# igashov/DiffLinker

Measured on NVIDIA H100. Metric: molecules/sec (T=500 denoising), higher is better.
Workload: dtype f32

## Files before the change

### difflinker_b200/csrc/common.cuh

```cuda
#pragma once
#include <cuda_runtime.h>
#include <stdint.h>

namespace dl {

constexpr int H = 128;
constexpr int MAX_DIN = 32;
constexpr int MAX_XHD = 16;

constexpr int OPT_TANH = 1;
constexpr int OPT_MEAN = 2;
constexpr int OPT_SIN = 4;
constexpr int N_SIN_FREQ = 6;
constexpr int N_SIN_FEAT = 4 * N_SIN_FREQ;
__device__ __forceinline__ float sin_freq(int k) { return __int_as_float(__float_as_int(0x1.aceeap-2f) + (k << 24)); }
__device__ __forceinline__ float sin_arg(float r, int k) { return __fmul_rn(__fsqrt_rn(__fadd_rn(r, 1e-8f)), sin_freq(k)); }
__device__ __forceinline__ float radial_rn(float dx, float dy, float dz) {
  return __fadd_rn(__fadd_rn(__fmul_rn(dx, dx), __fmul_rn(dy, dy)), __fmul_rn(dz, dz));
}

__device__ __forceinline__ void chain_wait() { asm volatile("griddepcontrol.wait;" ::: "memory"); }
__device__ __forceinline__ void chain_release() { asm volatile("griddepcontrol.launch_dependents;" ::: "memory"); }

inline bool& chain_overlap_enabled() { static bool on = true; return on; }

template <typename... KArgs, typename... Args>
inline cudaError_t launch_chain(void (*kernel)(KArgs...), dim3 grid, dim3 block, size_t smem, cudaStream_t st, Args&&... args) {
  cudaLaunchConfig_t cfg = {};
  cfg.gridDim = grid; cfg.blockDim = block; cfg.dynamicSmemBytes = smem; cfg.stream = st;
  cudaLaunchAttribute at[1];
  at[0].id = cudaLaunchAttributeProgrammaticStreamSerialization;
  at[0].val.programmaticStreamSerializationAllowed = chain_overlap_enabled() ? 1 : 0;
  cfg.attrs = at; cfg.numAttrs = 1;
  return cudaLaunchKernelEx(&cfg, kernel, KArgs(static_cast<Args&&>(args))...);
}

__device__ __forceinline__ float silu_f(float x) {
  float t, r;
  asm("ex2.approx.ftz.f32 %0, %1;" : "=f"(t) : "f"(x * -1.4426950408889634f));
  asm("rcp.approx.ftz.f32 %0, %1;" : "=f"(r) : "f"(1.0f + t));
  return x * r;
}

__device__ __forceinline__ float usig_f(float u) {
  float t, r;
  asm("ex2.approx.ftz.f32 %0, %1;" : "=f"(t) : "f"(u));
  asm("rcp.approx.ftz.f32 %0, %1;" : "=f"(r) : "f"(1.0f + t));
  return u * r;
}

__device__ __forceinline__ float2 fadd2(float2 a, float2 b) { return make_float2(__fadd_rn(a.x, b.x), __fadd_rn(a.y, b.y)); }
__device__ __forceinline__ float2 fmul2(float2 a, float2 b) { return make_float2(__fmul_rn(a.x, b.x), __fmul_rn(a.y, b.y)); }
__device__ __forceinline__ float2 ffma2(float2 a, float2 b, float2 c) { return make_float2(__fmaf_rn(a.x, b.x, c.x), __fmaf_rn(a.y, b.y, c.y)); }
__device__ __forceinline__ float ex2_approx(float x) { float y; asm("ex2.approx.ftz.f32 %0, %1;" : "=f"(y) : "f"(x)); return y; }
__device__ __forceinline__ float rcp_approx(float x) { float y; asm("rcp.approx.ftz.f32 %0, %1;" : "=f"(y) : "f"(x)); return y; }
__device__ __forceinline__ float2 sigmoid_pair_log2(float2 u) {
  const float2 den = fadd2(make_float2(ex2_approx(fminf(u.x, 63.0f)), ex2_approx(fminf(u.y, 63.0f))), make_float2(1.0f, 1.0f));
  const float r = rcp_approx(den.x * den.y);
  return fmul2(make_float2(r, r), make_float2(den.y, den.x));
}
__device__ __forceinline__ void usig4(float2 u01, float2 u23, float2& s01, float2& s23) {
  const float2 one = make_float2(1.0f, 1.0f);
  const float2 ab = fadd2(make_float2(ex2_approx(fminf(u01.x, 31.0f)), ex2_approx(fminf(u01.y, 31.0f))), one);
  const float2 cd = fadd2(make_float2(ex2_approx(fminf(u23.x, 31.0f)), ex2_approx(fminf(u23.y, 31.0f))), one);
  const float2 m = fmul2(ab, cd);
  const float r = rcp_approx(m.x * m.y);
  const float2 rm = fmul2(make_float2(r, r), make_float2(m.y, m.x));
  s01 = fmul2(u01, fmul2(rm, cd));
  s23 = fmul2(u23, fmul2(rm, ab));
}
__device__ __forceinline__ float2 usig2(float2 u) { return fmul2(u, sigmoid_pair_log2(u)); }
__device__ __forceinline__ float2 silu2(float2 x) {
  return fmul2(x, sigmoid_pair_log2(fmul2(x, make_float2(-1.4426950408889634f, -1.4426950408889634f))));
}

struct EdgeMlpW {
  const float* W1a_t;
  const float* W1b_t;
  const float* b1;
  const float* wd;
  const float* w0;
  const float* W2_t;
  const float* b2;
  const void* W2_tc;
  float w2_descale;
  float wdmax, w0max;
  const void* W1_tc;
  float w1_descale;
  const float* b1_u;
  const float* wd_u;
  const float* w0_u;
  const float* we;
  const float* we_u;
};

struct GclW : EdgeMlpW {
  const float* W3_t;
  const float* b3;
  const float* W4_t;
  const float* b4;
  const void* W3_tc;
  const void* W4_tc;
  float w3_descale, w4_descale;
};

struct EqW : EdgeMlpW {
  const float* w5;
};

struct ProjW {
  const float* W1a_t;
  const float* W1b_t;
  const float* b1;
};

struct Plan {
  const int* rowidx;
  const int* colidx;
  const int* xrowidx;
  const int* nr;
  const int* nc;
  const int* nxr;
  const int4* items;
  const int* n_items;
  const int* xmols;
  const int* n_xmols;
  const int4* xitems;
  const int* n_xitems;
};

struct Geom {
  int B, N;
  int F;
  int C;
  int D;
  int graph_type;
  float norm_constant;
  float normalization_factor;
};

}
```

### difflinker_b200/csrc/dl_engine.cu

```cuda
#include <cuda_fp16.h>
#include <cuda_runtime.h>

#include <algorithm>
#include <cmath>
#include <cstdarg>
#include <cstdio>
#include <cstdlib>
#include <cstring>
#include <ctime>
#include <map>
#include <string>
#include <vector>

#include "../../include/difflinker_b200.h"
#include "kernels_simt.cuh"
#include "kernels_tc.cuh"
#include "kernels_node_tc.cuh"
#include "kernels_retry.cuh"

using namespace dl;

static thread_local char g_err[1024] = "";
static void set_err(const char* fmt, ...) {
  va_list ap;
  va_start(ap, fmt);
  vsnprintf(g_err, sizeof(g_err), fmt, ap);
  va_end(ap);
}

#define CK(call)                                                                          \
  do {                                                                                    \
    cudaError_t _e = (call);                                                              \
    if (_e != cudaSuccess) {                                                              \
      set_err("%s:%d %s -> %s", __FILE__, __LINE__, #call, cudaGetErrorString(_e));       \
      return DL_ERR_CUDA;                                                                 \
    }                                                                                     \
  } while (0)

namespace {

struct Workspace {
  int B = 0, N = 0;
  float *nm = nullptr, *x0 = nullptr, *xa = nullptr, *xb = nullptr, *h = nullptr, *ABg = nullptr, *ABc = nullptr,
        *agg = nullptr, *z = nullptr, *ABgmax = nullptr, *ABcmax = nullptr, *eps = nullptr;
  int* cls = nullptr;
  int *nbr = nullptr, *recs = nullptr, *xrecs = nullptr, *n_recs = nullptr;
  float4 *x04 = nullptr, *xa4 = nullptr, *xb4 = nullptr;
  int *rowidx = nullptr, *colidx = nullptr, *xrowidx = nullptr, *nr = nullptr, *nc = nullptr, *nxr = nullptr,
      *n_items = nullptr, *xmols = nullptr, *n_xmols = nullptr, *n_xitems = nullptr;
  int4* items = nullptr;
  int4* xitems = nullptr;
  int* tile_ctr = nullptr;
  unsigned long long* seeds = nullptr;
  std::vector<void*> allocs;
};

struct HostStage {
  size_t cap = 0;
  char* buf = nullptr;
};

struct KernelTimes {
  bool on = false;
  struct Rec { const char* label; cudaEvent_t a, b; };
  std::vector<Rec> pending;
  std::map<std::string, std::pair<double, long>> acc;
  void begin(cudaStream_t st, const char* label) {
    if (!on) return;
    cudaStreamCaptureStatus cap = cudaStreamCaptureStatusNone;
    cudaStreamIsCapturing(st, &cap);
    if (cap != cudaStreamCaptureStatusNone) return;
    Rec r{label, nullptr, nullptr};
    cudaEventCreate(&r.a); cudaEventCreate(&r.b);
    cudaEventRecord(r.a, st);
    pending.push_back(r);
  }
  void end(cudaStream_t st) {
    if (!on || pending.empty() || pending.back().b == nullptr) return;
    cudaStreamCaptureStatus cap = cudaStreamCaptureStatusNone;
    cudaStreamIsCapturing(st, &cap);
    if (cap != cudaStreamCaptureStatusNone) return;
    cudaEventRecord(pending.back().b, st);
  }
  void collect(cudaStream_t st) {
    if (!on || pending.empty()) return;
    cudaStreamSynchronize(st);
    for (auto& r : pending) {
      float ms = 0.f;
      if (cudaEventElapsedTime(&ms, r.a, r.b) == cudaSuccess) { auto& a = acc[r.label]; a.first += ms; a.second += 1; }
      cudaEventDestroy(r.a); cudaEventDestroy(r.b);
    }
    pending.clear();
  }
  void report() {
    if (!on || acc.empty()) return;
    double tot = 0;
    for (auto& kv : acc) tot += kv.second.first;
    for (auto& kv : acc)
      fprintf(stderr, "[dl times] %-22s %6ld launches  avg %8.2f us  share %5.1f%%\n", kv.first.c_str(), kv.second.second,
              1e3 * kv.second.first / kv.second.second, 100.0 * kv.second.first / tot);
  }
};

}

struct dl_engine {
  dl_config cfg{};
  dl_egnn_options opts{};
  int D = 0;
  int num_sms = 0;
  int max_threads_per_sm = 2048;
  int slice_B_full = 0, slice_b0 = 0;
  int start_step = -1;
  float start_alpha = 0.f, start_sigma = 0.f;
  std::vector<int32_t> starts_t0;
  std::vector<float> starts_alpha, starts_sigma;
  HostStage start_rows;
  int resamplings = 1, resample_T = 0;
  std::vector<float> jump;
  std::vector<dl_step_coef> coef_passes;
  int64_t mol_steps = 0;
  bool finalized = false;
  std::map<std::string, std::vector<float>> raw;
  float* wblob = nullptr;
  __half* wblob_tc = nullptr;
  std::vector<GclW> gcl;
  std::vector<EqW> eq;
  const float *We_t = nullptr, *be = nullptr, *Wo = nullptr, *bo = nullptr;
  Workspace ws;
  Workspace ws_sub;
  HostStage sub_rows;
  HostStage hashes;
  bool ring_set = false;
  unsigned long long ring_allowed = 0;
  HostStage ring_masks;
  int ring_B = 0;
  HostStage anchors;
  bool anchors_set = false;
  int anchors_B = 0, anchors_N = 0;
  cudaEvent_t ev_r0 = nullptr, ev_r1 = nullptr, ev_g0 = nullptr, ev_g1 = nullptr;
  float retry_ms = 0.f;
  cudaStream_t loop_stream = nullptr;
  cudaEvent_t ev_in = nullptr, ev_out = nullptr, ev_t0 = nullptr, ev_t1 = nullptr;
  float* coef_dev = nullptr;
  int coef_cap = 0;
  int* step_ctr = nullptr;
  int64_t launches = 0;
  HostStage stage;
  KernelTimes times;
  bool use_tc = false;
  const int8_t* last_edge_mask = nullptr;
  const float* last_linker_mask = nullptr;
  int last_B = 0, last_N = 0;
};

namespace {

int edges_in(const dl_engine* e) { return e->opts.sin_embedding ? N_SIN_FEAT : 2; }

#define TIMED(label, stream, stmt) do { e->times.begin(stream, label); stmt; e->times.end(stream); } while (0)

struct ExpectedParam {
  std::string name;
  int64_t numel;
};

std::vector<ExpectedParam> expected_params(const dl_config& c, int edges_in) {
  const int D = c.in_node_nf + c.context_node_nf + (c.condition_time ? 1 : 0);
  const int Hh = c.hidden_nf;
  std::vector<ExpectedParam> v;
  v.push_back({"dynamics.embedding.weight", (int64_t)Hh * D});
  v.push_back({"dynamics.embedding.bias", Hh});
  v.push_back({"dynamics.embedding_out.weight", (int64_t)D * Hh});
  v.push_back({"dynamics.embedding_out.bias", D});
  char buf[160];
  for (int l = 0; l < c.n_layers; ++l) {
    for (int s = 0; s < c.inv_sublayers; ++s) {
      snprintf(buf, sizeof(buf), "dynamics.e_block_%d.gcl_%d.", l, s);
      std::string p(buf);
      v.push_back({p + "edge_mlp.0.weight", (int64_t)Hh * (2 * Hh + edges_in)});
      v.push_back({p + "edge_mlp.0.bias", Hh});
      v.push_back({p + "edge_mlp.2.weight", (int64_t)Hh * Hh});
      v.push_back({p + "edge_mlp.2.bias", Hh});
      v.push_back({p + "node_mlp.0.weight", (int64_t)Hh * 2 * Hh});
      v.push_back({p + "node_mlp.0.bias", Hh});
      v.push_back({p + "node_mlp.2.weight", (int64_t)Hh * Hh});
      v.push_back({p + "node_mlp.2.bias", Hh});
    }
    snprintf(buf, sizeof(buf), "dynamics.e_block_%d.gcl_equiv.", l);
    std::string p(buf);
    v.push_back({p + "coord_mlp.0.weight", (int64_t)Hh * (2 * Hh + edges_in)});
    v.push_back({p + "coord_mlp.0.bias", Hh});
    v.push_back({p + "coord_mlp.2.weight", (int64_t)Hh * Hh});
    v.push_back({p + "coord_mlp.2.bias", Hh});
    v.push_back({p + "coord_mlp.4.weight", Hh});
  }
  return v;
}

using RawWeights = std::map<std::string, std::vector<float>>;

struct Packer {
  std::vector<float> blob;
  std::vector<__half> tc;
  std::vector<std::pair<const float**, size_t>> fields;
  std::vector<std::pair<const void**, size_t>> tc_fields;
  void add(const float** field, const std::vector<float>& seg) {
    while (blob.size() % 4) blob.push_back(0.f);
    fields.push_back({field, blob.size()});
    blob.insert(blob.end(), seg.begin(), seg.end());
  }
  void add_tc(const void** field, size_t off) { tc_fields.push_back({field, off}); }
  void point(const float* base, const __half* tc_base) const {
    for (auto& f : fields) *f.first = base + f.second;
    for (auto& f : tc_fields) *f.first = tc_base + f.second;
  }
};

std::vector<float> transpose_block(const std::vector<float>& W, int out, int in_stride, int c0, int k) {
  std::vector<float> t((size_t)k * out);
  for (int o = 0; o < out; ++o)
    for (int i = 0; i < k; ++i) t[(size_t)i * out + o] = W[(size_t)o * in_stride + c0 + i];
  return t;
}
std::vector<float> column(const std::vector<float>& W, int out, int in_stride, int c) {
  std::vector<float> t(out);
  for (int o = 0; o < out; ++o) t[o] = W[(size_t)o * in_stride + c];
  return t;
}

void pack_edge_mlp(Packer& pk, EdgeMlpW& w, const RawWeights& raw, const std::string& p, int in1) {
  const auto& W1 = raw.at(p + "0.weight");
  pk.add(&w.W1a_t, transpose_block(W1, H, in1, 0, H));
  pk.add(&w.W1b_t, transpose_block(W1, H, in1, H, H));
  pk.add(&w.b1, raw.at(p + "0.bias"));
  pk.add(&w.wd, column(W1, H, in1, 2 * H));
  pk.add(&w.W2_t, transpose_block(raw.at(p + "2.weight"), H, H, 0, H));
  pk.add(&w.b2, raw.at(p + "2.bias"));
}

void pack_gcl(Packer& pk, GclW& w, const RawWeights& raw, const std::string& p, int in1) {
  pack_edge_mlp(pk, w, raw, p + "edge_mlp.", in1);
  pk.add(&w.W3_t, transpose_block(raw.at(p + "node_mlp.0.weight"), H, 2 * H, 0, 2 * H));
  pk.add(&w.b3, raw.at(p + "node_mlp.0.bias"));
  pk.add(&w.W4_t, transpose_block(raw.at(p + "node_mlp.2.weight"), H, H, 0, H));
  pk.add(&w.b4, raw.at(p + "node_mlp.2.bias"));
}

void pack_edge_mlp_denoiser(Packer& pk, EdgeMlpW& w, const RawWeights& raw, const std::string& p, bool sin_embedding) {
  const int IN1 = 2 * H + (sin_embedding ? N_SIN_FEAT : 2);
  auto scaled = [](const std::vector<float>& v) { std::vector<float> o(v.size()); for (size_t i = 0; i < v.size(); ++i) o[i] = (float)((double)v[i] * tc::NEG_LOG2E); return o; };
  auto absmax = [](const std::vector<float>& v) { float m = 0.f; for (float x : v) m = std::max(m, std::fabs(x)); return m; };
  const auto& W1 = raw.at(p + "0.weight");
  const std::vector<float> wd = column(W1, H, IN1, 2 * H), w0 = column(W1, H, IN1, 2 * H + 1);
  pk.add(&w.w0, w0);
  pk.add_tc(&w.W2_tc, tc::pack_w2(raw.at(p + "2.weight"), pk.tc, &w.w2_descale));
  pk.add_tc(&w.W1_tc, tcn::pack_blocks(scaled(W1), IN1, 2, pk.tc, &w.w1_descale));
  pk.add(&w.b1_u, scaled(raw.at(p + "0.bias")));
  pk.add(&w.wd_u, scaled(wd));
  pk.add(&w.w0_u, scaled(w0));
  w.wdmax = absmax(wd); w.w0max = absmax(w0);
  if (sin_embedding) {
    const std::vector<float> we = transpose_block(W1, H, IN1, 2 * H, N_SIN_FEAT);
    pk.add(&w.we, we);
    pk.add(&w.we_u, scaled(we));
    w.wdmax = 0.f; w.w0max = 0.f;
    for (int k = 0; k < N_SIN_FEAT; ++k) w.wdmax += absmax(std::vector<float>(we.begin() + k * H, we.begin() + (k + 1) * H));
  }
}

template <typename T>
dl_status upload_blob(const std::vector<T>& host, T** dev) {
  if (*dev) cudaFree(*dev);
  *dev = nullptr;
  CK(cudaMalloc((void**)dev, std::max<size_t>(host.size(), 1) * sizeof(T)));
  CK(cudaMemcpy(*dev, host.data(), host.size() * sizeof(T), cudaMemcpyHostToDevice));
  return DL_OK;
}

template <typename T>
dl_status dev_alloc(Workspace& ws, T** p, size_t count) {
  void* q = nullptr;
  CK(cudaMalloc(&q, std::max<size_t>(count, 1) * sizeof(T)));
  ws.allocs.push_back(q);
  *p = reinterpret_cast<T*>(q);
  return DL_OK;
}

void free_workspace(Workspace& ws) {
  for (void* p : ws.allocs) cudaFree(p);
  ws = Workspace();
}

dl_status ensure_workspace(dl_engine* e, int B, int N) {
  Workspace& ws = e->ws;
  if (ws.B == B && ws.N == N) return DL_OK;
  free_workspace(ws);
  const size_t n = (size_t)B * N;
  const int xd = 3 + e->cfg.in_node_nf;
  dl_status s;
#define WSA(field, cnt) if ((s = dev_alloc(ws, &ws.field, (cnt))) != DL_OK) return s
  WSA(nm, n); WSA(x0, n * 3); WSA(xa, n * 3); WSA(xb, n * 3); WSA(h, n * H); WSA(ABg, n * 2 * H); WSA(ABc, n * 2 * H);
  WSA(agg, n * H); WSA(z, n * xd); WSA(eps, n * xd); WSA(cls, n); WSA(x04, n); WSA(xa4, n); WSA(xb4, n); WSA(ABgmax, n * 2); WSA(ABcmax, n * 2);
  WSA(rowidx, n); WSA(colidx, n); WSA(xrowidx, n); WSA(nr, B); WSA(nc, B); WSA(nxr, B); WSA(n_items, 1);
  WSA(xmols, B); WSA(n_xmols, 1); WSA(items, n); WSA(xitems, n); WSA(n_xitems, 1); WSA(tile_ctr, 64); WSA(seeds, B);
  if (e->use_tc && e->cfg.graph_type != 0) { WSA(nbr, n * N); WSA(recs, n * CUT_REC); WSA(xrecs, n * CUT_REC); WSA(n_recs, 2); }
#undef WSA
  ws.B = B; ws.N = N;
  return DL_OK;
}

Plan make_plan(const Workspace& ws) {
  Plan p;
  p.rowidx = ws.rowidx; p.colidx = ws.colidx; p.xrowidx = ws.xrowidx; p.nr = ws.nr; p.nc = ws.nc; p.nxr = ws.nxr;
  p.items = ws.items; p.n_items = ws.n_items; p.xmols = ws.xmols; p.n_xmols = ws.n_xmols;
  p.xitems = ws.xitems; p.n_xitems = ws.n_xitems;
  return p;
}

Geom make_geom(const dl_engine* e, int B, int N) {
  Geom g;
  g.B = B; g.N = N; g.F = e->cfg.in_node_nf; g.C = e->cfg.context_node_nf; g.D = e->D;
  g.graph_type = e->cfg.graph_type; g.norm_constant = e->cfg.norm_constant;
  g.normalization_factor = e->cfg.normalization_factor;
  return g;
}

#define LAUNCH_CHECK()                                                                    \
  do {                                                                                    \
    cudaError_t _e = cudaGetLastError();                                                  \
    if (_e != cudaSuccess) {                                                              \
      set_err("%s:%d kernel launch -> %s", __FILE__, __LINE__, cudaGetErrorString(_e));   \
      return DL_ERR_CUDA;                                                                 \
    }                                                                                     \
  } while (0)

constexpr int PLAN_MAX_N = 48 * 1024 / (2 * (int)sizeof(int));

dl_status build_plan(Workspace& ws, int B, int N, int graph_type, const int8_t* node_mask, const float* linker_mask,
                     const int8_t* edge_mask, int tile_edges, int max_rows, cudaStream_t st) {
  if (N > PLAN_MAX_N) {
    set_err("N = %d exceeds the work plan's limit of %d rows per molecule", N, PLAN_MAX_N);
    return DL_ERR_UNSUPPORTED;
  }
  CK(cudaMemsetAsync(ws.agg, 0, (size_t)B * N * H * sizeof(float), st));
  k_plan_mol<<<B, 256, 2 * N * sizeof(int), st>>>(N, graph_type, edge_mask, node_mask, linker_mask, ws.rowidx,
                                                  ws.colidx, ws.xrowidx, ws.nr, ws.nc, ws.nxr);
  LAUNCH_CHECK();
  k_plan_items<<<1, 1, 0, st>>>(B, tile_edges, max_rows, 1, max_rows, ws.nr, ws.nc, ws.nxr, ws.items, ws.n_items, ws.xmols,
                                ws.n_xmols, ws.xitems, ws.n_xitems);
  LAUNCH_CHECK();
  return DL_OK;
}

dl_status build_forward_plan(dl_engine* e, int B, int N, const int8_t* node_mask, const float* linker_mask,
                             const int8_t* edge_mask, cudaStream_t st) {
  const dl_status s = build_plan(e->ws, B, N, e->cfg.graph_type, node_mask, linker_mask, edge_mask,
                                 e->use_tc ? tc::TN : ET, e->use_tc ? tc::MAXR : MAXR, st);
  if (s == DL_OK) e->launches += 2;
  return s;
}

struct FwdIO {
  const float* xh = nullptr; const float* t = nullptr; int t_numel = 0; float* out = nullptr;
  const int8_t* node_mask = nullptr; const float* linker_mask = nullptr; const int8_t* edge_mask = nullptr;
  const float* context = nullptr; int* nan_flags = nullptr;
  bool sampler = false; bool inpaint = false; const float* xh0 = nullptr; const float* upd_linker_mask = nullptr;
  const float* fragment_mask = nullptr; const float* noise = nullptr; float* chain = nullptr;
  NoiseRng rng{};
  int T = 0; float norm0 = 1.f, norm1 = 1.f, bias1 = 0.f;
  RowStarts rows{};
  int R = 1; const float* jump = nullptr;
};

ProjW proj_of(const EdgeMlpW& w) { return ProjW{w.W1a_t, w.W1b_t, w.b1}; }

EdgeArgs edge_args(const dl_engine* e, const EdgeMlpW& w, bool coord, const int8_t* edge_mask, const float* linker_mask,
                   const float* x, const float4* x4, float* x_out = nullptr, float4* x4_out = nullptr,
                   const float* w5 = nullptr) {
  const Workspace& ws = e->ws;
  const float ksc = e->use_tc ? 1.4426950408889634f : 1.0f;
  EdgeArgs ea{};
  ea.AB = coord ? ws.ABc : ws.ABg; ea.ABmax = coord ? ws.ABcmax : ws.ABgmax;
  ea.w2_descale = w.w2_descale; ea.wdmax = w.wdmax * ksc; ea.w0max = w.w0max * ksc;
  ea.x = x; ea.x0 = ws.x0; ea.x4 = x4; ea.x04 = ws.x04; ea.x4_out = x4_out;
  ea.edge_mask = edge_mask; ea.cls = ws.cls; ea.nm = ws.nm; ea.linker_mask = linker_mask;
  ea.W2_t = w.W2_t; ea.b2 = w.b2; ea.wd = e->use_tc ? w.wd_u : w.wd; ea.w0 = e->use_tc ? w.w0_u : w.w0; ea.w5 = w5;
  ea.plan = make_plan(ws); ea.agg = coord ? nullptr : ws.agg; ea.x_out = x_out; ea.nbr = ws.nbr;
  ea.recs = coord ? ws.xrecs : ws.recs;
  ea.n_recs = coord && ws.n_recs ? ws.n_recs + 1 : ws.n_recs;
  ea.coords_range = e->opts.coords_range;
  ea.we = e->use_tc ? w.we_u : w.we;
  return ea;
}

int edge_opt(const dl_engine* e, bool coord) {
  return (coord && e->opts.tanh ? OPT_TANH : 0) | (e->opts.aggregation == DL_AGGR_MEAN ? OPT_MEAN : 0) |
         (e->opts.sin_embedding ? OPT_SIN : 0);
}

struct NodeConsumer { const EdgeMlpW* w; float* AB; float* ABmax; };
int node_consumers(const dl_engine* e, int l, int s, NodeConsumer c[2]) {
  const int L = e->cfg.n_layers, S = e->cfg.inv_sublayers;
  const Workspace& ws = e->ws;
  if (s + 1 < S) { c[0] = {&e->gcl[l * S + s + 1], ws.ABg, ws.ABgmax}; return 1; }
  c[0] = {&e->eq[l], ws.ABc, ws.ABcmax};
  if (l + 1 == L) return 1;
  c[1] = {&e->gcl[(l + 1) * S], ws.ABg, ws.ABgmax};
  return 2;
}

tcn::NodeTcArgs node_tc_args(const dl_engine* e, const GclW& w, int l, int s) {
  const Workspace& ws = e->ws;
  tcn::NodeTcArgs ta{};
  ta.h = ws.h; ta.agg = ws.agg; ta.nm = ws.nm; ta.proj_only = s < 0;
  ta.w3 = reinterpret_cast<const __half*>(w.W3_tc); ta.w4 = reinterpret_cast<const __half*>(w.W4_tc);
  ta.b3 = w.b3; ta.b4 = w.b4; ta.w3_descale = w.w3_descale; ta.w4_descale = w.w4_descale;
  NodeConsumer c[2];
  ta.n_proj = node_consumers(e, l, s, c);
  for (int i = 0; i < ta.n_proj; ++i) {
    ta.pw[i] = reinterpret_cast<const __half*>(c[i].w->W1_tc); ta.pb1[i] = c[i].w->b1_u;
    ta.p_descale[i] = c[i].w->w1_descale; ta.AB[i] = c[i].AB; ta.ABmax[i] = c[i].ABmax;
  }
  ta.tile_nodes = tcn::pick_tile_nodes(ws.B * ws.N, e->num_sms);
  return ta;
}

template <bool COORD, int OPT = 0>
void launch_edge_simt(int opt, int num_sms, const Geom& gm, const EdgeArgs& ea, cudaStream_t st) {
  if constexpr (OPT <= (OPT_TANH | OPT_MEAN | OPT_SIN)) {
    if constexpr (COORD || !(OPT & OPT_TANH))
      if (opt == OPT) { k_edge_simt<COORD, ACT_SILU, OPT><<<num_sms, 256, EDGE_SIMT_SMEM, st>>>(gm, ea); return; }
    launch_edge_simt<COORD, OPT + 1>(opt, num_sms, gm, ea, st);
  }
}

template <bool COORD, int OPT = 0>
cudaError_t opt_in_edge_simt() {
  if constexpr (OPT > (OPT_TANH | OPT_MEAN | OPT_SIN)) {
    return cudaSuccess;
  } else {
    if constexpr (COORD || !(OPT & OPT_TANH)) {
      const cudaError_t err = cudaFuncSetAttribute(k_edge_simt<COORD, ACT_SILU, OPT>, cudaFuncAttributeMaxDynamicSharedMemorySize,
                                                   (int)EDGE_SIMT_SMEM);
      if (err != cudaSuccess) return err;
    }
    return opt_in_edge_simt<COORD, OPT + 1>();
  }
}

dl_status launch_edge(dl_engine* e, const Geom& gm, const EdgeArgs& ea, bool coord, const void* w2_tc, cudaStream_t st) {
  const int opt = edge_opt(e, coord);
  if (e->use_tc) {
    dl_status s = tc::launch_edge_tc(gm, ea, coord, opt, w2_tc, e->num_sms, st);
    if (s != DL_OK) { set_err("no tensor-core edge kernel for graph type %d with options %d", gm.graph_type, opt); return s; }
  } else if (coord) {
    launch_edge_simt<true>(opt, e->num_sms, gm, ea, st);
  } else {
    launch_edge_simt<false>(opt, e->num_sms, gm, ea, st);
  }
  LAUNCH_CHECK();
  e->launches += 1;
  return DL_OK;
}

dl_status enqueue_forward(dl_engine* e, int B, int N, const FwdIO& io, cudaStream_t st) {
  Workspace& ws = e->ws;
  const Geom gm = make_geom(e, B, N);
  const int n = B * N;
  const int L = e->cfg.n_layers, S = e->cfg.inv_sublayers;
  const int node_blocks = (n + NODE_TM - 1) / NODE_TM;
  const size_t node_smem = 3 * NODE_TM * LDX * sizeof(float);

  PrepArgs pa{};
  pa.xh = io.sampler ? ws.z : io.xh;
  pa.node_mask = io.node_mask; pa.linker_mask = io.linker_mask;
  pa.t = io.t; pa.t_numel = io.t_numel; pa.context = io.context;
  pa.We_t = e->We_t; pa.be = e->be; pa.proj = proj_of(e->gcl[0]);
  pa.nm = ws.nm; pa.x0 = ws.x0; pa.x = ws.xa; pa.x04 = e->use_tc ? ws.x04 : nullptr; pa.x4 = e->use_tc ? ws.xa4 : nullptr; pa.cls = ws.cls; pa.h = ws.h;
  pa.AB = e->use_tc ? nullptr : ws.ABg; pa.ABmax = ws.ABgmax;
  pa.coef = io.sampler ? e->coef_dev : nullptr;
  pa.step_prep = io.sampler ? e->step_ctr : nullptr;
  pa.step_fin = io.sampler ? e->step_ctr + 1 : nullptr;
  TIMED("k_prep", st, (launch_chain(k_prep, dim3(node_blocks), dim3(256), 0, st, gm, pa)));
  LAUNCH_CHECK();
  e->launches += 1;
  if (e->use_tc) {
    const tcn::NodeTcArgs ta = node_tc_args(e, e->gcl[0], 0, -1);
    TIMED("k_node_tc(proj only)", st, (tcn::launch_node(n, ta, st)));
    LAUNCH_CHECK();
    e->launches += 1;
  }

  if (ws.nbr != nullptr) {
    CK(cudaMemsetAsync(ws.n_recs, 0, 2 * sizeof(int), st));
    k_nbr<<<B, 512, (size_t)N * CUT_SMEM_PER_NODE, st>>>(N, e->cfg.graph_type, ws.x04, ws.cls, ws.rowidx, ws.colidx,
                                                        ws.xrowidx, ws.nr, ws.nc, ws.nxr, ws.nbr, ws.recs, ws.xrecs,
                                                        ws.n_recs);
    LAUNCH_CHECK();
    e->launches += 1;
  }

  float* xin = ws.xa;
  float* xout = ws.xb;
  float4* xin4 = ws.xa4;
  float4* xout4 = ws.xb4;
  e->last_edge_mask = io.edge_mask; e->last_linker_mask = io.linker_mask; e->last_B = B; e->last_N = N;
  for (int l = 0; l < L; ++l) {
    for (int s = 0; s < S; ++s) {
      const GclW& w = e->gcl[l * S + s];
      const EdgeArgs ea = edge_args(e, w, false, io.edge_mask, io.linker_mask, xin, xin4);
      e->times.begin(st, "edge GCL");
      dl_status st2 = launch_edge(e, gm, ea, false, w.W2_tc, st);
      e->times.end(st);
      if (st2 != DL_OK) return st2;

      if (e->use_tc) {
        const tcn::NodeTcArgs ta = node_tc_args(e, w, l, s);
        TIMED(ta.n_proj == 2 ? "k_node_tc(2 proj)" : "k_node_tc(1 proj)", st, (tcn::launch_node(n, ta, st)));
      } else {
        NodeArgs na{};
        na.h = ws.h; na.agg = ws.agg; na.nm = ws.nm; na.W3_t = w.W3_t; na.b3 = w.b3; na.W4_t = w.W4_t; na.b4 = w.b4;
        NodeConsumer c[2];
        const int n_proj = node_consumers(e, l, s, c);
        na.proj1 = proj_of(*c[0].w); na.AB1 = c[0].AB; na.ABmax1 = c[0].ABmax;
        if (n_proj == 2) { na.proj2 = proj_of(*c[1].w); na.AB2 = c[1].AB; na.ABmax2 = c[1].ABmax; }
        k_node<ACT_SILU><<<node_blocks, 256, node_smem, st>>>(n, na);
      }
      LAUNCH_CHECK();
      e->launches += 1;
    }
    k_copy_x<<<(n * 3 + 255) / 256, 256, 0, st>>>(n * 3, xin, xout, e->use_tc ? xin4 : nullptr, xout4);
    LAUNCH_CHECK();
    e->launches += 1;
    const EqW& w = e->eq[l];
    const EdgeArgs ea = edge_args(e, w, true, io.edge_mask, io.linker_mask, xin, xin4, xout, xout4, w.w5);
    e->times.begin(st, "edge COORD");
    dl_status st2 = launch_edge(e, gm, ea, true, w.W2_tc, st);
    e->times.end(st);
    if (st2 != DL_OK) return st2;
    std::swap(xin, xout);
    std::swap(xin4, xout4);
  }

  FinishArgs fa{};
  fa.h = ws.h; fa.x = xin; fa.x0 = ws.x0; fa.nm = ws.nm; fa.Wo = e->Wo; fa.bo = e->bo;
  fa.nan_flags = io.nan_flags;
  const bool fused_update = io.sampler && !io.inpaint;
  fa.out = fused_update ? nullptr : (io.sampler ? ws.eps : io.out);
  if (fused_update) {
    fa.z = ws.z; fa.fragment_mask = io.fragment_mask; fa.linker_mask = io.linker_mask; fa.noise = io.noise; fa.rng = io.rng;
    fa.coef = e->coef_dev; fa.step_fin = e->step_ctr + 1; fa.step_prep = e->step_ctr; fa.T = io.T;
    fa.norm0 = io.norm0; fa.norm1 = io.norm1; fa.bias1 = io.bias1; fa.chain = io.chain; fa.rows = io.rows;
  } else if (io.sampler) {
    fa.tag_step = e->step_ctr + (io.R > 1 ? 2 : 1);
  }
  const bool per_mol = io.rng.on == NOISE_PER_MOLECULE;
  TIMED("k_finish", st, (launch_chain(per_mol ? k_finish<true> : k_finish<false>, dim3((n + 15) / 16), dim3(256), 0, st, gm, fa)));
  LAUNCH_CHECK();
  e->launches += 1;
  if (e->cfg.centering || io.inpaint) {
    InpaintArgs ia{};
    ia.mode = io.inpaint ? 1 : 0;
    ia.eps = io.inpaint ? ws.eps : io.out; ia.nm = ws.nm; ia.z = ws.z; ia.xh0 = io.xh0;
    ia.fragment_mask = io.fragment_mask; ia.linker_mask = io.upd_linker_mask; ia.noise = io.noise; ia.rng = io.rng;
    ia.coef = e->coef_dev;
    ia.step_prep = e->step_ctr; ia.step_fin = e->step_ctr + 1; ia.T = io.T;
    ia.norm0 = io.norm0; ia.norm1 = io.norm1; ia.bias1 = io.bias1; ia.chain = io.chain;
    ia.R = io.R; ia.jump = io.jump; ia.step_tag = e->step_ctr + 2;
    if (io.R > 1) {
      if (per_mol) k_inpaint<true, true><<<B, 256, 0, st>>>(gm, ia);
      else k_inpaint<false, true><<<B, 256, 0, st>>>(gm, ia);
    } else if (per_mol) k_inpaint<true><<<B, 256, 0, st>>>(gm, ia);
    else k_inpaint<false><<<B, 256, 0, st>>>(gm, ia);
    LAUNCH_CHECK();
    e->launches += 1;
  }
  return DL_OK;
}

dl_status check_shapes(const dl_engine* e, int B, int N) {
  if (!e || !e->finalized) { set_err("engine not finalized (dl_finalize_weights)"); return DL_ERR_INVALID; }
  if (B <= 0 || N <= 0) { set_err("B and N must be positive (got %d, %d)", B, N); return DL_ERR_INVALID; }
  if ((int64_t)B * N * N > (int64_t)1 << 40) { set_err("B*N*N too large"); return DL_ERR_INVALID; }
  if (e->use_tc && e->cfg.graph_type != 0 && N > 4000) {
    set_err("cut-off graphs: N = %d exceeds the neighbour-list kernel's shared-memory staging (N <= 4000)", N);
    return DL_ERR_INVALID;
  }
  return DL_OK;
}

size_t align256(size_t v) { return (v + 255) & ~(size_t)255; }

struct StageLayout {
  struct Buf { const void* src; size_t bytes, off; bool used; };
  std::vector<Buf> bufs;
  size_t total = 0;
  char* base = nullptr;
  int add(const void* src, size_t bytes, bool used) {
    bufs.push_back({src, bytes, total, used});
    total += used ? align256(bytes) : 0;
    return (int)bufs.size() - 1;
  }
  int in(const void* src, size_t bytes) { return add(src, bytes, src != nullptr); }
  int out(size_t bytes) { return add(nullptr, bytes, true); }
  template <typename T> T* at(int i) const { return bufs[i].used ? reinterpret_cast<T*>(base + bufs[i].off) : nullptr; }
};

dl_status stage_inputs(HostStage& sg, StageLayout& sl, cudaStream_t st) {
  if (sg.cap < sl.total) {
    if (sg.buf) cudaFree(sg.buf);
    sg.buf = nullptr; sg.cap = 0;
    CK(cudaMalloc((void**)&sg.buf, sl.total));
    sg.cap = sl.total;
  }
  sl.base = sg.buf;
  for (const auto& b : sl.bufs)
    if (b.src) CK(cudaMemcpyAsync(sl.base + b.off, b.src, b.bytes, cudaMemcpyHostToDevice, st));
  return DL_OK;
}

dl_status stage_results(void* out, const void* d_out, size_t bytes, const int32_t* d_flags, int B, int32_t* nan_flags,
                        cudaStream_t st) {
  std::vector<int32_t> flags(B);
  CK(cudaMemcpyAsync(out, d_out, bytes, cudaMemcpyDeviceToHost, st));
  CK(cudaMemcpyAsync(flags.data(), d_flags, B * 4, cudaMemcpyDeviceToHost, st));
  CK(cudaStreamSynchronize(st));
  bool any = false;
  for (int i = 0; i < B; ++i) { any |= flags[i] != 0; if (nan_flags) nan_flags[i] = flags[i]; }
  return any ? DL_NAN_DETECTED : DL_OK;
}

dl_status check_slice(const dl_engine* e, int B) {
  if (e->slice_B_full > 0 && e->slice_b0 + B > e->slice_B_full) {
    set_err("batch slice [%d, %d) exceeds the full batch %d", e->slice_b0, e->slice_b0 + B, e->slice_B_full);
    return DL_ERR_INVALID;
  }
  return DL_OK;
}

dl_status check_sampler(const dl_engine* e, int sampler, int T, int keep_frames, bool has_draws, const float* xh,
                        const int8_t* node_mask, const float* fragment_mask, const float* linker_mask, const float* context,
                        const dl_step_coef* coef, const float* norm, const float* chain) {
  if (sampler != DL_SAMPLER_LINKER && sampler != DL_SAMPLER_INPAINT) { set_err("unknown sampler %d", sampler); return DL_ERR_INVALID; }
  if ((sampler == DL_SAMPLER_INPAINT) != (e->cfg.centering != 0)) { set_err("the inpainting sampler needs a model built with centering=1 (and vice versa)"); return DL_ERR_INVALID; }
  if (!xh || !node_mask || !fragment_mask || !linker_mask || !has_draws || !coef || !norm || !chain) {
    set_err("null argument"); return DL_ERR_INVALID;
  }
  if (T < 1 || keep_frames < 1 || keep_frames > T) { set_err("need 1 <= keep_frames <= T"); return DL_ERR_INVALID; }
  if (e->cfg.context_node_nf > 0 && !context) { set_err("context required"); return DL_ERR_INVALID; }
  return DL_OK;
}

uint64_t sampler_draws(int sampler, int T, int R = 1) {
  return sampler == DL_SAMPLER_INPAINT ? 1 + (uint64_t)T * (3 * R - 1) + 2 : (uint64_t)T + 2;
}

int call_resamplings(const dl_engine* e, int sampler, int T) {
  if (e->resamplings == 1) return 1;
  if (sampler != DL_SAMPLER_INPAINT) { set_err("resampling (dl_set_resamplings) takes DL_SAMPLER_INPAINT only"); return 0; }
  if (T != e->resample_T) {
    set_err("dl_set_resamplings was given the jump coefficients of T = %d; the call samples T = %d", e->resample_T, T);
    return 0;
  }
  return e->resamplings;
}

int loop_steps(const dl_engine* e, int T) {
  if (e && !e->starts_t0.empty()) return *std::max_element(e->starts_t0.begin(), e->starts_t0.end());
  return e && e->start_step >= 0 ? e->start_step : T;
}

struct SubBatchScope {
  dl_engine* e;
  const int8_t* edge_mask;
  const float* linker_mask;
  int B, N;
  int64_t mol_steps;
  explicit SubBatchScope(dl_engine* e_)
      : e(e_), edge_mask(e_->last_edge_mask), linker_mask(e_->last_linker_mask), B(e_->last_B), N(e_->last_N),
        mol_steps(e_->mol_steps) { swap(); }
  ~SubBatchScope() {
    swap();
    e->last_edge_mask = edge_mask; e->last_linker_mask = linker_mask; e->last_B = B; e->last_N = N;
    e->mol_steps = mol_steps;
  }
  void swap() { std::swap(e->ws, e->ws_sub); std::swap(e->ev_t0, e->ev_r0); std::swap(e->ev_t1, e->ev_r1); }
};

struct RowOrder {
  const float *xh, *fragment_mask, *linker_mask, *context, *alpha, *sigma;
  const int8_t *node_mask, *edge_mask;
  RowStarts rs;
  std::vector<int> active;
};

dl_status order_rows(dl_engine* e, int B, int N, int Tl, const float* xh, const int8_t* node_mask, const float* fragment_mask,
                     const float* linker_mask, const int8_t* edge_mask, const float* context, const unsigned long long* seeds,
                     cudaStream_t st, RowOrder& ro) {
  const std::vector<int32_t>& t0 = e->starts_t0;
  std::vector<int> order(B), lag(B);
  std::vector<float> al(B), sg(B);
  for (int b = 0; b < B; ++b) order[b] = b;
  std::stable_sort(order.begin(), order.end(), [&](int a, int b) { return t0[a] > t0[b]; });
  for (int i = 0; i < B; ++i) {
    lag[i] = Tl - t0[order[i]]; al[i] = e->starts_alpha[order[i]]; sg[i] = e->starts_sigma[order[i]];
  }
  ro.active.resize(Tl + 1);
  for (int r = 0; r <= Tl; ++r) ro.active[r] = (int)(std::upper_bound(lag.begin(), lag.end(), r) - lag.begin());
  const bool fc_em = edge_mask && e->cfg.graph_type == DL_GRAPH_FC;
  const int xd = 3 + e->cfg.in_node_nf, C = e->cfg.context_node_nf;
  const size_t n = (size_t)B * N;
  StageLayout sl;
  const int i_src = sl.in(order.data(), B * sizeof(int)), i_lag = sl.in(lag.data(), B * sizeof(int)),
            i_al = sl.in(al.data(), B * sizeof(float)), i_sg = sl.in(sg.data(), B * sizeof(float)), i_xh = sl.out(n * xd * 4),
            i_nm = sl.out(n), i_fm = sl.out(n * 4), i_lm = sl.out(n * 4), i_em = sl.add(nullptr, n * N, fc_em),
            i_ctx = sl.add(nullptr, n * C * 4, context != nullptr && C > 0);
  dl_status s = stage_inputs(e->start_rows, sl, st);
  if (s != DL_OK) return s;
  RowGatherArgs ga{};
  ga.rows = sl.at<const int>(i_src); ga.N = N; ga.xd = xd; ga.C = C; ga.attempt = 0;
  ga.xh = xh; ga.fragment_mask = fragment_mask; ga.linker_mask = linker_mask; ga.context = sl.at<float>(i_ctx) ? context : nullptr;
  ga.node_mask = node_mask; ga.edge_mask = fc_em ? edge_mask : nullptr; ga.seeds = seeds;
  ga.s_xh = sl.at<float>(i_xh); ga.s_fragment_mask = sl.at<float>(i_fm); ga.s_linker_mask = sl.at<float>(i_lm);
  ga.s_context = sl.at<float>(i_ctx); ga.s_node_mask = sl.at<int8_t>(i_nm); ga.s_edge_mask = sl.at<int8_t>(i_em);
  ga.s_seeds = e->ws.seeds;
  k_gather_rows<false><<<B, 256, 0, st>>>(ga);
  LAUNCH_CHECK();
  e->launches += 1;
  ro.xh = ga.s_xh; ro.fragment_mask = ga.s_fragment_mask; ro.linker_mask = ga.s_linker_mask; ro.context = ga.s_context;
  ro.node_mask = ga.s_node_mask; ro.edge_mask = ga.s_edge_mask;
  ro.alpha = sl.at<const float>(i_al); ro.sigma = sl.at<const float>(i_sg);
  ro.rs = RowStarts{sl.at<const int>(i_lag), sl.at<const int>(i_src), (int)n};
  return DL_OK;
}

dl_status capture_step(dl_engine* e, int Bp, int N, const FwdIO& io, cudaStream_t st, cudaGraph_t* graph) {
  CK(cudaStreamBeginCapture(st, cudaStreamCaptureModeThreadLocal));
  const dl_status s = enqueue_forward(e, Bp, N, io, st);
  const cudaError_t ce = cudaStreamEndCapture(st, graph);
  if (s != DL_OK) { if (*graph) cudaGraphDestroy(*graph); *graph = nullptr; return s; }
  if (ce != cudaSuccess) { set_err("cudaStreamEndCapture -> %s", cudaGetErrorString(ce)); return DL_ERR_CUDA; }
  return DL_OK;
}

}

extern "C" {

const char* dl_version(void) { return "difflinker_b200 0.1 (sm_90a)"; }
const char* dl_last_error(void) { return g_err; }

dl_status dl_create(const dl_config* cfg, dl_engine** out) { return dl_create_ex(cfg, nullptr, out); }

dl_status dl_create_ex(const dl_config* cfg, const dl_egnn_options* opts, dl_engine** out) {
  if (!cfg || !out) { set_err("null argument"); return DL_ERR_INVALID; }
  const dl_egnn_options o = opts ? *opts : dl_egnn_options{0, 15.0f, 0, DL_AGGR_SUM};
  if (o.sin_embedding != 0 && o.sin_embedding != 1) { set_err("sin_embedding must be 0 or 1 (got %d)", o.sin_embedding); return DL_ERR_INVALID; }
  if (o.tanh != 0 && o.tanh != 1) { set_err("tanh must be 0 or 1 (got %d)", o.tanh); return DL_ERR_INVALID; }
  if (o.aggregation != DL_AGGR_SUM && o.aggregation != DL_AGGR_MEAN) { set_err("unknown aggregation %d", o.aggregation); return DL_ERR_INVALID; }
  if (!std::isfinite(o.coords_range)) { set_err("coords_range must be finite"); return DL_ERR_INVALID; }
  if (cfg->hidden_nf != H) { set_err("hidden_nf must be %d (got %d)", H, cfg->hidden_nf); return DL_ERR_UNSUPPORTED; }
  if (cfg->n_dims != 3) { set_err("n_dims must be 3"); return DL_ERR_UNSUPPORTED; }
  const int D = cfg->in_node_nf + cfg->context_node_nf + (cfg->condition_time ? 1 : 0);
  if (D > MAX_DIN || cfg->in_node_nf < 1 || 3 + cfg->in_node_nf > MAX_XHD) {
    set_err("unsupported feature widths F=%d C=%d", cfg->in_node_nf, cfg->context_node_nf);
    return DL_ERR_UNSUPPORTED;
  }
  if (cfg->n_layers < 1 || cfg->inv_sublayers < 1) { set_err("n_layers/inv_sublayers must be >= 1"); return DL_ERR_INVALID; }
  if (cfg->graph_type < 0 || cfg->graph_type > 3) { set_err("bad graph_type"); return DL_ERR_INVALID; }
  if (cfg->graph_type != DL_GRAPH_FC && cfg->context_node_nf < 2) {
    set_err("pocket graphs need fragment_only/pocket_only context columns"); return DL_ERR_INVALID;
  }
  int ndev = 0;
  CK(cudaGetDeviceCount(&ndev));
  if (cfg->device < 0 || cfg->device >= ndev) { set_err("device %d not available (%d devices)", cfg->device, ndev); return DL_ERR_INVALID; }
  CK(cudaSetDevice(cfg->device));
  cudaDeviceProp prop;
  CK(cudaGetDeviceProperties(&prop, cfg->device));
  if (prop.major != 9 || prop.minor != 0) {
    set_err("difflinker_b200 is built for sm_90a only; device is sm_%d%d", prop.major, prop.minor);
    return DL_ERR_UNSUPPORTED;
  }
  dl_engine* e = new dl_engine();
  e->cfg = *cfg;
  e->opts = o;
  e->D = D;
  e->num_sms = prop.multiProcessorCount;
  e->max_threads_per_sm = prop.maxThreadsPerMultiProcessor;
  e->use_tc = tc::AVAILABLE && cfg->edge_impl != DL_EDGE_SIMT;
  CK(cudaStreamCreateWithFlags(&e->loop_stream, cudaStreamNonBlocking));
  CK(cudaEventCreateWithFlags(&e->ev_in, cudaEventDisableTiming));
  CK(cudaEventCreateWithFlags(&e->ev_out, cudaEventDisableTiming));
  CK(cudaEventCreate(&e->ev_t0));
  CK(cudaEventCreate(&e->ev_t1));
  CK(cudaEventCreate(&e->ev_r0));
  CK(cudaEventCreate(&e->ev_r1));
  CK(cudaEventCreate(&e->ev_g0));
  CK(cudaEventCreate(&e->ev_g1));
  CK(cudaMalloc((void**)&e->step_ctr, 3 * sizeof(int)));
  CK(cudaFuncSetAttribute(k_node<ACT_SILU>, cudaFuncAttributeMaxDynamicSharedMemorySize, 3 * NODE_TM * LDX * sizeof(float)));
  CK(opt_in_edge_simt<true>());
  CK(opt_in_edge_simt<false>());
  CK(cudaFuncSetAttribute(k_nbr, cudaFuncAttributeMaxDynamicSharedMemorySize, 4000 * CUT_SMEM_PER_NODE));
  if (getenv("DL_TIME_KERNELS")) e->times.on = true;
  if (const char* v = getenv("DL_WAIT_MODE")) { const int m = atoi(v); cudaMemcpyToSymbol(tc::c_wait_mode, &m, sizeof(int)); }
  if (const char* v = getenv("DL_CHAIN_OVERLAP")) chain_overlap_enabled() = atoi(v) != 0;
  dl_status s = tc::configure();
  if (s == DL_OK) s = tcn::configure_node();
  if (s != DL_OK) { set_err("cudaFuncSetAttribute failed for the tensor-core kernels"); delete e; return s; }
  *out = e;
  return DL_OK;
}

dl_status dl_destroy(dl_engine* e) {
  if (!e) return DL_OK;
  e->times.report();
  cudaSetDevice(e->cfg.device);
  cudaDeviceSynchronize();
  free_workspace(e->ws);
  free_workspace(e->ws_sub);
  if (e->sub_rows.buf) cudaFree(e->sub_rows.buf);
  if (e->start_rows.buf) cudaFree(e->start_rows.buf);
  if (e->hashes.buf) cudaFree(e->hashes.buf);
  if (e->ring_masks.buf) cudaFree(e->ring_masks.buf);
  if (e->anchors.buf) cudaFree(e->anchors.buf);
  if (e->wblob) cudaFree(e->wblob);
  if (e->wblob_tc) cudaFree(e->wblob_tc);
  if (e->coef_dev) cudaFree(e->coef_dev);
  if (e->step_ctr) cudaFree(e->step_ctr);
  if (e->stage.buf) cudaFree(e->stage.buf);
  if (e->loop_stream) cudaStreamDestroy(e->loop_stream);
  if (e->ev_in) cudaEventDestroy(e->ev_in);
  if (e->ev_out) cudaEventDestroy(e->ev_out);
  if (e->ev_t0) cudaEventDestroy(e->ev_t0);
  if (e->ev_t1) cudaEventDestroy(e->ev_t1);
  for (cudaEvent_t ev : {e->ev_r0, e->ev_r1, e->ev_g0, e->ev_g1}) if (ev) cudaEventDestroy(ev);
// ... 1108 lines not shown
```

### difflinker_b200/csrc/kernels_node_tc.cuh

```cuda
#pragma once
#include "kernels_tc.cuh"

namespace dl {
namespace tcn {

using namespace dl::tc;

constexpr int TM = 128;
constexpr int X_LBO = TM * 16 + 16;
constexpr int X_BYTES = KC * X_LBO;
constexpr int HALF_BYTES = 8 * W_LBO;
constexpr int STAGE_BYTES = 2 * HALF_BYTES;
constexpr int BLOCK_BYTES = 2 * W_BYTES;
constexpr int N_RING = 2;
constexpr int N_OFF_WS = 4 * X_BYTES;
constexpr int N_OFF_MISC = N_OFF_WS + N_RING * STAGE_BYTES;
constexpr int N_OFF_BAR = N_OFF_MISC + 128 * 4 + 64;
constexpr int N_SMEM_BYTES = N_OFF_BAR + 64 + 1024;
static_assert(N_SMEM_BYTES <= 232448, "k_node_tc shared memory");
constexpr int NW = 8;
constexpr int W_NLOADER = NW;
constexpr int NODE_TC_THREADS = 32 * (NW + 1);

struct NodeTcArgs {
  float* h;
  const float* agg;
  const float* nm;
  const __half* w3;
  const __half* w4;
  const float *b3, *b4;
  float w3_descale, w4_descale;
  int tile_nodes;
  int proj_only;
  int n_proj;
  const __half* pw[2];
  const float* pb1[2];
  float p_descale[2];
  float* AB[2];
  float* ABmax[2];
};

__device__ __forceinline__ float pow2_scale_for(float bound) {
  float sc = 1.0f;
  if (!(bound <= F16_TARGET)) {
    const int ex = ((__float_as_int(bound) >> 23) & 0xff) - 127;
    sc = __int_as_float(max(127 + 13 - ex, 1) << 23);
  }
  return sc;
}

__device__ __forceinline__ void workers_sync() { asm volatile("bar.sync 1, %0;" ::"n"(32 * NW) : "memory"); }

__device__ __forceinline__ void store_elem(uint8_t* xhi, uint8_t* xlo, int c, int n, float v) {
  const __half hi = __float2half_rn(v);
  const __half lo = __float2half_rn(v - __half2float(hi));
  const int off = (c >> 3) * X_LBO + n * 16 + (c & 7) * 2;
  *reinterpret_cast<__half*>(xhi + off) = hi;
  *reinterpret_cast<__half*>(xlo + off) = lo;
}

__global__ void __launch_bounds__(NODE_TC_THREADS, 1) k_node_tc(int n_total, NodeTcArgs a) {
  extern __shared__ uint8_t smem_raw[];
  uint8_t* sm = smem_raw + ((1024u - (smem_u32(smem_raw) & 1023u)) & 1023u);
  const uint32_t sbase = smem_u32(sm);
  const int tid = threadIdx.x, warp = tid >> 5, lane = tid & 31;
  const int tile = a.tile_nodes > 0 ? a.tile_nodes : TM;
  const int g0 = blockIdx.x * tile;
  const int n_live = min(tile, n_total - g0);

  const uint32_t bar_full = sbase + N_OFF_BAR, bar_empty = bar_full + 8 * N_RING;
  uint8_t* xa_hi = sm; uint8_t* xa_lo = xa_hi + X_BYTES;
  uint8_t* xb_hi = sm + 2 * X_BYTES; uint8_t* xb_lo = xb_hi + X_BYTES;
  float* nms = reinterpret_cast<float*>(sm + N_OFF_MISC);
  int* tilemax = reinterpret_cast<int*>(sm + N_OFF_MISC + 512);

  if (tid == 0) {
    for (int i = 0; i < N_RING; ++i) { mbar_init(bar_full + 8 * i, 1); mbar_init(bar_empty + 8 * i, NW); }
    fence_barrier_init();
  }
  if (tid < 16) tilemax[tid] = 0;
  __syncthreads();

  const int blk0 = a.proj_only ? 3 : 0;
  const int n_blocks = 3 + 2 * a.n_proj - blk0;
  const int n_half = 2 * n_blocks;

  if (warp == W_NLOADER) {
    if (lane == 0) {
      for (int i = 0; i < n_half; ++i) {
        const int s = i % N_RING, blk = (i >> 1) + blk0, hf = i & 1;
        if (i >= N_RING) mbar_wait(bar_empty + 8 * s, ((i - N_RING) / N_RING) & 1);
        const __half* base = blk < 2 ? a.w3 + (size_t)blk * (BLOCK_BYTES / 2)
                             : blk == 2 ? a.w4
                                        : a.pw[(blk - 3) >> 1] + (size_t)((blk - 3) & 1) * (BLOCK_BYTES / 2);
        const uint8_t* src = reinterpret_cast<const uint8_t*>(base);
        const uint32_t dst = sbase + N_OFF_WS + s * STAGE_BYTES;
        mbar_expect_tx(bar_full + 8 * s, STAGE_BYTES);
        bulk_g2s(dst, src + hf * HALF_BYTES, HALF_BYTES, bar_full + 8 * s);
        bulk_g2s(dst + HALF_BYTES, src + W_BYTES + hf * HALF_BYTES, HALF_BYTES, bar_full + 8 * s);
      }
    }
    return;
  }

  chain_wait();
  if (tid == 0) chain_release();
  if (tid < TM) nms[tid] = tid < n_live ? a.nm[g0 + tid] : 0.f;

  const int g = warp >> 2, q = lane & 3;
  const int c0 = 64 * g + 16 * (warp & 3) + (lane >> 2);
  int tm_calls = 0;
  auto tile_max = [&](float mx) -> float {
#pragma unroll
    for (int o = 16; o > 0; o >>= 1) mx = fmaxf(mx, __shfl_xor_sync(0xffffffffu, mx, o));
    int* slot = tilemax + (tm_calls++ & 15);
    if (lane == 0) atomicMax(slot, __float_as_int(mx));
    workers_sync();
    return __int_as_float(*slot);
  };
  auto operand_ready = [&]() {
    fence_proxy_async();
    workers_sync();
  };
  int hb = 0;
  float d[64];
#pragma unroll
  for (int i = 0; i < 64; ++i) d[i] = 0.f;
  auto gemm = [&](const uint8_t* xop, int n_blk_half, bool accumulate) {
    for (int k = 0; k < n_blk_half; ++k, ++hb) {
      const int s = hb % N_RING, hf = hb & 1;
      mbar_wait(bar_full + 8 * s, (hb / N_RING) & 1);
      const uint32_t xh = smem_u32(xop) + (8 * hf) * X_LBO, xl = xh + X_BYTES;
      const uint32_t wh = sbase + N_OFF_WS + s * STAGE_BYTES + g * 1024, wl = wh + HALF_BYTES;
      gemm_3xf16(d, wh, wl, W_LBO, xh, xl, X_LBO, 2 * X_LBO, 4, accumulate || k > 0);
      __syncwarp();
      if (lane == 0) mbar_arrive(bar_empty + 8 * s);
    }
  };

  auto load_rows = [&](float scale) -> float {
    float mx = 0.f;
#pragma unroll 1
    for (int rb = warp; rb < TM; rb += 4 * NW) {
      float4 hv[4], av[4];
#pragma unroll
      for (int j = 0; j < 4; ++j) {
        const int r = rb + NW * j;
        hv[j] = make_float4(0, 0, 0, 0); av[j] = hv[j];
        if (r < n_live) {
          hv[j] = *reinterpret_cast<const float4*>(a.h + (size_t)(g0 + r) * H + lane * 4);
          if (!a.proj_only) av[j] = __ldg(reinterpret_cast<const float4*>(a.agg + (size_t)(g0 + r) * H + lane * 4));
        }
      }
#pragma unroll
      for (int j = 0; j < 4; ++j) {
        const int r = rb + NW * j;
        mx = fmaxf(mx, fmaxf(fmaxf(fabsf(hv[j].x), fabsf(hv[j].y)), fmaxf(fabsf(hv[j].z), fabsf(hv[j].w))));
        mx = fmaxf(mx, fmaxf(fmaxf(fabsf(av[j].x), fabsf(av[j].y)), fmaxf(fabsf(av[j].z), fabsf(av[j].w))));
        const int off = (lane >> 1) * X_LBO + r * 16 + (lane & 1) * 8;
        uint2 hi, lo;
        split2(hv[j].x * scale, hv[j].y * scale, hi.x, lo.x); split2(hv[j].z * scale, hv[j].w * scale, hi.y, lo.y);
        *reinterpret_cast<uint2*>(xa_hi + off) = hi; *reinterpret_cast<uint2*>(xa_lo + off) = lo;
        split2(av[j].x * scale, av[j].y * scale, hi.x, lo.x); split2(av[j].z * scale, av[j].w * scale, hi.y, lo.y);
        *reinterpret_cast<uint2*>(xb_hi + off) = hi; *reinterpret_cast<uint2*>(xb_lo + off) = lo;
      }
    }
    return mx;
  };

  float s1 = 1.f, s2 = 1.f, s3 = 1.f;
#pragma unroll 1
  for (int pass = 0; pass < 2; ++pass) {
    const float mx = load_rows(s1);
    if (pass == 1) break;
    s1 = pow2_scale_for(tile_max(mx));
    if (s1 == 1.0f) break;
  }
  operand_ready();

  if (a.proj_only) {
    s3 = s1;
  } else {
    gemm(xa_hi, 2, false);
    gemm(xb_hi, 2, true);
    workers_sync();
    const float2 bias3 = make_float2(__ldg(a.b3 + c0), __ldg(a.b3 + c0 + 8));
    const float ds1 = a.w3_descale / s1;
#pragma unroll 1
    for (int pass = 0; pass < 2; ++pass) {
      float mx = 0.f;
#pragma unroll
      for (int j = 0; j < 16; ++j)
#pragma unroll
        for (int u = 0; u < 4; ++u) {
          const float v = fmaf(d[4 * j + u], ds1, (u & 2) ? bias3.y : bias3.x);
          mx = fmaxf(mx, fabsf(v));
          store_elem(xb_hi, xb_lo, c0 + (u & 2) * 4, 8 * j + 2 * q + (u & 1), silu_f(v) * s2);
        }
      if (pass == 1) break;
      s2 = pow2_scale_for(tile_max(mx));
      if (s2 == 1.0f) break;
    }
    operand_ready();
    gemm(xb_hi, 2, false);
    const float2 bias4 = make_float2(__ldg(a.b4 + c0), __ldg(a.b4 + c0 + 8));
    const float ds2 = a.w4_descale / s2;
    float mx = 0.f;
#pragma unroll
    for (int j = 0; j < 16; ++j)
#pragma unroll
      for (int u = 0; u < 4; ++u) {
        const int n = 8 * j + 2 * q + (u & 1), c = c0 + (u & 2) * 4;
        float* hp = a.h + (size_t)(g0 + n) * H + c;
        const float hv = n < n_live ? *hp : 0.f;
        const float o = (hv + fmaf(d[4 * j + u], ds2, (u & 2) ? bias4.y : bias4.x)) * nms[n];
        if (n < n_live) *hp = o;
        mx = fmaxf(mx, fabsf(o));
        d[4 * j + u] = o;
        store_elem(xa_hi, xa_lo, c, n, o);
      }
    s3 = pow2_scale_for(tile_max(mx));
    if (s3 != 1.0f) {
#pragma unroll
      for (int j = 0; j < 16; ++j)
#pragma unroll
        for (int u = 0; u < 4; ++u) store_elem(xa_hi, xa_lo, c0 + (u & 2) * 4, 8 * j + 2 * q + (u & 1), d[4 * j + u] * s3);
    }
    operand_ready();
  }

  for (int p = 0; p < a.n_proj; ++p) {
#pragma unroll 1
    for (int pt = 0; pt < 2; ++pt) {
      gemm(xa_hi, 2, false);
      const float2 bias = pt == 0 ? make_float2(__ldg(a.pb1[p] + c0), __ldg(a.pb1[p] + c0 + 8)) : make_float2(0.f, 0.f);
      float* ab = a.AB[p] + (size_t)g0 * 2 * H + pt * H;
      const float ds = a.p_descale[p] / s3;
      float mx = 0.f;
#pragma unroll
      for (int j = 0; j < 16; ++j)
#pragma unroll
        for (int u = 0; u < 4; ++u) {
          const int n = 8 * j + 2 * q + (u & 1);
          const float o = fmaf(d[4 * j + u], ds, (u & 2) ? bias.y : bias.x);
          if (n < n_live) { ab[(size_t)n * 2 * H + c0 + (u & 2) * 4] = o; mx = fmaxf(mx, fabsf(o)); }
        }
      const float tmx = tile_max(mx);
      if (tid < n_live) a.ABmax[p][(size_t)(g0 + tid) * 2 + pt] = tmx;
    }
  }
}

inline size_t pack_blocks(const std::vector<float>& W, int in_stride, int nblk, std::vector<__half>& blob,
                          float* descale) {
  while (blob.size() % 64) blob.push_back(__float2half(0.f));
  const size_t off = blob.size();
  const size_t per = 2 * (size_t)KC * H * 8;
  blob.resize(off + nblk * per);
  float mx = 0.f;
  for (int c = 0; c < H; ++c)
    for (int k = 0; k < nblk * H; ++k) mx = std::max(mx, std::fabs(W[(size_t)c * in_stride + k]));
  int ex = 0;
  if (mx > 0.f && std::isfinite(mx)) { std::frexp(mx, &ex); ex -= 1; }
  const int sh = std::min(std::max(13 - ex, -40), 40);
  const float scale = std::ldexp(1.0f, sh);
  *descale = std::ldexp(1.0f, -sh);
  for (int b = 0; b < nblk; ++b)
    for (int kc = 0; kc < KC; ++kc)
      for (int c = 0; c < H; ++c)
        for (int u = 0; u < 8; ++u) {
          const float v = W[(size_t)c * in_stride + b * H + kc * 8 + u] * scale;
          const __half hi = __float2half_rn(v);
          const __half lo = __float2half_rn(v - __half2float(hi));
          blob[off + b * per + ((size_t)kc * H + c) * 8 + u] = hi;
          blob[off + b * per + (size_t)KC * H * 8 + ((size_t)kc * H + c) * 8 + u] = lo;
        }
  return off;
}

inline int pick_tile_nodes(int n, int num_sms) {
  const int per = (n + num_sms - 1) / std::max(num_sms, 1);
  return std::min(TM, std::max(8, (per + 7) & ~7));
}

inline dl_status configure_node() {
  if (cudaFuncSetAttribute(k_node_tc, cudaFuncAttributeMaxDynamicSharedMemorySize, N_SMEM_BYTES) != cudaSuccess) return DL_ERR_CUDA;
  return DL_OK;
}

inline void launch_node(int n, const NodeTcArgs& ta, cudaStream_t st) {
  const int grid = (n + ta.tile_nodes - 1) / ta.tile_nodes;
  launch_chain(k_node_tc, dim3(grid), dim3(NODE_TC_THREADS), N_SMEM_BYTES, st, n, ta);
}

}
}
```

### difflinker_b200/csrc/kernels_simt.cuh

```cuda
#pragma once
#include <curand_kernel.h>

#include "common.cuh"

namespace dl {

__global__ void k_plan_mol(int N, int graph_type, const int8_t* __restrict__ edge_mask,
                           const int8_t* __restrict__ node_mask, const float* __restrict__ linker_mask,
                           int* __restrict__ rowidx, int* __restrict__ colidx, int* __restrict__ xrowidx,
                           int* __restrict__ nr, int* __restrict__ nc, int* __restrict__ nxr) {
  extern __shared__ int sm_plan[];
  int* rowlive = sm_plan;
  int* collive = sm_plan + N;
  const int b = blockIdx.x;
  const int tid = threadIdx.x, lane = tid & 31, warp = tid >> 5, nwarp = blockDim.x >> 5;
  for (int i = tid; i < N; i += blockDim.x) { rowlive[i] = 0; collive[i] = 0; }
  __syncthreads();
  if ((graph_type == 0 || graph_type == 4) && edge_mask != nullptr) {
    const int8_t* em = edge_mask + (size_t)b * N * N;
    for (int i = warp; i < N; i += nwarp) {
      int any = 0;
      for (int j = lane; j < N; j += 32) {
        int v = em[(size_t)i * N + j];
        if (v != 0) { any = 1; collive[j] = 1; }
      }
      any = __any_sync(0xffffffffu, any);
      if (lane == 0 && any) rowlive[i] = 1;
    }
  } else if (graph_type == 0 || graph_type == 4) {
    for (int i = tid; i < N; i += blockDim.x) { rowlive[i] = 1; collive[i] = 1; }
  } else {
    for (int i = tid; i < N; i += blockDim.x) {
      int v = node_mask[(size_t)b * N + i] != 0;
      rowlive[i] = v; collive[i] = v;
    }
  }
  __syncthreads();
  if (tid == 0) {
    int a = 0, c = 0, x = 0;
    for (int i = 0; i < N; ++i) {
      if (rowlive[i]) {
        rowidx[(size_t)b * N + a++] = i;
        if (linker_mask == nullptr || linker_mask[(size_t)b * N + i] != 0.0f) xrowidx[(size_t)b * N + x++] = i;
      }
      if (collive[i]) colidx[(size_t)b * N + c++] = i;
    }
    nr[b] = a; nc[b] = c; nxr[b] = x;
  }
}

__global__ void k_plan_items(int B, int tile_edges, int max_rows, int col_pad, int max_rows_gcl, const int* __restrict__ nr,
                             const int* __restrict__ nc, const int* __restrict__ nxr, int4* __restrict__ items,
                             int* __restrict__ n_items, int* __restrict__ xmols, int* __restrict__ n_xmols,
                             int4* __restrict__ xitems, int* __restrict__ n_xitems, int n_cta = 0,
                             int* __restrict__ cta_begin = nullptr, int* __restrict__ xcta_begin = nullptr) {
  if (threadIdx.x != 0 || blockIdx.x != 0) return;
  int cnt = 0, xc = 0, xi = 0;
  for (int b = 0; b < B; ++b) {
    int r = nr[b], c = nc[b];
    if (r > 0 && c > 0) {
      const int cp = (c + col_pad - 1) / col_pad * col_pad;
      int per = cp >= tile_edges ? 1 : tile_edges / cp;
      if (per > max_rows_gcl) per = max_rows_gcl;
      for (int r0 = 0; r0 < r; r0 += per) items[cnt++] = make_int4(b, r0, min(per, r - r0), c);
    }
    if (nxr[b] > 0 && c > 0) {
      xmols[xc++] = b;
      int per;
      if (col_pad > 1) {
        const int cp = (c + col_pad - 1) / col_pad * col_pad;
        per = cp >= tile_edges ? 1 : tile_edges / cp;
        if (per > max_rows_gcl) per = max_rows_gcl;
      } else {
        per = c >= tile_edges ? 1 : tile_edges / c;
        if (per > max_rows) per = max_rows;
      }
      for (int r0 = 0; r0 < nxr[b]; r0 += per) xitems[xi++] = make_int4(b, r0, min(per, nxr[b] - r0), c);
    }
  }
  *n_items = cnt;
  *n_xmols = xc;
  *n_xitems = xi;
  if (n_cta > 0 && cta_begin != nullptr) {
    for (int pass = 0; pass < 2; ++pass) {
      const int4* list = pass == 0 ? items : xitems;
      const int total = pass == 0 ? cnt : xi;
      int* out = pass == 0 ? cta_begin : xcta_begin;
      if (out == nullptr) continue;
      long long sum = 0;
      for (int k = 0; k < total; ++k) sum += (long long)list[k].z * ((list[k].w + col_pad - 1) / col_pad * col_pad) + 32;
      long long run = 0;
      int c = 0;
      out[0] = 0;
      for (int k = 0; k < total; ++k) {
        while (c + 1 < n_cta && run * n_cta >= (long long)(c + 1) * sum) out[++c] = k;
        run += (long long)list[k].z * ((list[k].w + col_pad - 1) / col_pad * col_pad) + 32;
      }
      while (c < n_cta) out[++c] = total;
    }
  }
}

constexpr int ACT_SILU = 0, ACT_RELU = 1;
template <int ACT>
__device__ __forceinline__ float act_f(float x) { return ACT == ACT_RELU ? fmaxf(x, 0.f) : silu_f(x); }

constexpr int NODE_TM = 32;
constexpr int LDX = 132;

template <int K>
__device__ __forceinline__ void warp_gemm_4x4(const float* __restrict__ xs, const float* __restrict__ Wt, int lane,
                                              float (&acc)[4][4]) {
#pragma unroll 2
  for (int k = 0; k < K; k += 4) {
    float4 w[4], x[4];
#pragma unroll
    for (int q = 0; q < 4; ++q) w[q] = __ldg(reinterpret_cast<const float4*>(Wt + (size_t)(k + q) * H + lane * 4));
#pragma unroll
    for (int r = 0; r < 4; ++r) x[r] = *reinterpret_cast<const float4*>(xs + r * LDX + k);
#pragma unroll
    for (int r = 0; r < 4; ++r) {
      const float xv[4] = {x[r].x, x[r].y, x[r].z, x[r].w};
#pragma unroll
      for (int q = 0; q < 4; ++q) {
        acc[r][0] = fmaf(xv[q], w[q].x, acc[r][0]);
        acc[r][1] = fmaf(xv[q], w[q].y, acc[r][1]);
        acc[r][2] = fmaf(xv[q], w[q].z, acc[r][2]);
        acc[r][3] = fmaf(xv[q], w[q].w, acc[r][3]);
      }
    }
  }
}

__device__ __forceinline__ void zero_acc(float (&acc)[4][4]) {
#pragma unroll
  for (int r = 0; r < 4; ++r)
#pragma unroll
    for (int c = 0; c < 4; ++c) acc[r][c] = 0.f;
}

__device__ __forceinline__ float warp_absmax4(const float (&v)[4]) {
  float m = fmaxf(fmaxf(fabsf(v[0]), fabsf(v[1])), fmaxf(fabsf(v[2]), fabsf(v[3])));
#pragma unroll
  for (int o = 16; o > 0; o >>= 1) m = fmaxf(m, __shfl_xor_sync(0xffffffffu, m, o));
  return m;
}

__device__ __forceinline__ void project_ab(const float* hs_warp, const ProjW& pw, float* __restrict__ AB,
                                           float* __restrict__ ABmax, int g0, int n_total, int warp, int lane) {
  float acc[4][4];
  zero_acc(acc);
  warp_gemm_4x4<H>(hs_warp, pw.W1a_t, lane, acc);
  const float4 bb = __ldg(reinterpret_cast<const float4*>(pw.b1 + lane * 4));
#pragma unroll
  for (int r = 0; r < 4; ++r) {
    int g = g0 + warp * 4 + r;
    const float o[4] = {acc[r][0] + bb.x, acc[r][1] + bb.y, acc[r][2] + bb.z, acc[r][3] + bb.w};
    const float mx = warp_absmax4(o);
    if (g < n_total) {
      *reinterpret_cast<float4*>(AB + (size_t)g * 2 * H + lane * 4) = make_float4(o[0], o[1], o[2], o[3]);
      if (lane == 0) ABmax[(size_t)g * 2] = mx;
    }
  }
  zero_acc(acc);
  warp_gemm_4x4<H>(hs_warp, pw.W1b_t, lane, acc);
#pragma unroll
  for (int r = 0; r < 4; ++r) {
    int g = g0 + warp * 4 + r;
    const float mx = warp_absmax4(acc[r]);
    if (g < n_total) {
      *reinterpret_cast<float4*>(AB + (size_t)g * 2 * H + H + lane * 4) =
          make_float4(acc[r][0], acc[r][1], acc[r][2], acc[r][3]);
      if (lane == 0) ABmax[(size_t)g * 2 + 1] = mx;
    }
  }
}

struct PrepArgs {
  const float* xh;
  const int8_t* node_mask;
  const float* linker_mask;
  const float* t;
  int t_numel;
  const float* context;
  const float* We_t;
  const float* be;
  ProjW proj;
  float* nm;
  float* x0;
  float* x;
  float4* x04;
  float4* x4;
  int* cls;
  float* h;
  float* AB;
  float* ABmax;
  const float* coef;
  const int* step_prep;
  int* step_fin;
};

__global__ void __launch_bounds__(256) k_prep(Geom gm, PrepArgs a) {
  __shared__ __align__(16) float hs[NODE_TM * LDX];
  __shared__ float hin[NODE_TM][MAX_DIN];
  const int tid = threadIdx.x, lane = tid & 31, warp = tid >> 5;
  const int n_total = gm.B * gm.N;
  const int g0 = blockIdx.x * NODE_TM;
  const int xd = 3 + gm.F;
  int step = 0;
  chain_wait();
  chain_release();
  if (a.step_prep != nullptr) {
    step = *a.step_prep;
    if (blockIdx.x == 0 && tid == 0) *a.step_fin = step;
  }
  for (int idx = tid; idx < NODE_TM * MAX_DIN; idx += 256) {
    int r = idx / MAX_DIN, d = idx % MAX_DIN;
    int g = g0 + r;
    float v = 0.f;
    if (g < n_total && d < gm.D) {
      float m = (float)a.node_mask[g];
      if (d < gm.F) {
        v = a.xh[(size_t)g * xd + 3 + d] * m;
      } else if (d == gm.F && gm.D > gm.F + gm.C) {
        if (a.coef != nullptr) v = a.coef[(size_t)step * 8 + 0];
        else v = a.t[a.t_numel == 1 ? 0 : g / gm.N];
      } else {
        int cidx = d - (gm.D - gm.C);
        v = a.context[(size_t)g * gm.C + cidx];
      }
    }
    hin[r][d] = v;
  }
  if (tid < NODE_TM) {
    int g = g0 + tid;
    if (g < n_total) {
      float m = (float)a.node_mask[g];
      a.nm[g] = m;
      for (int d = 0; d < 3; ++d) {
        float v = a.xh[(size_t)g * xd + d] * m;
        a.x0[(size_t)g * 3 + d] = v;
        a.x[(size_t)g * 3 + d] = v;
        if (a.x4 != nullptr) {
          reinterpret_cast<float*>(a.x04 + g)[d] = v;
          reinterpret_cast<float*>(a.x4 + g)[d] = v;
        }
      }
      if (gm.graph_type >= 1 && gm.graph_type <= 3) {
        int valid = m != 0.f;
        int pk = a.context[(size_t)g * gm.C + gm.C - 1] != 0.f;
        int fr = a.context[(size_t)g * gm.C + gm.C - 2] != 0.f;
        int lk = a.linker_mask != nullptr ? (a.linker_mask[g] != 0.f) : 0;
        int c = 0;
        if (valid) {
          if (gm.graph_type == 1) c = 1;
          else c = (lk || fr) ? 1 : (pk ? 2 : 3);
        }
        a.cls[g] = c;
      }
    }
  }
  __syncthreads();
  {
    float acc[4][4];
    zero_acc(acc);
    for (int d = 0; d < gm.D; ++d) {
      const float4 w = __ldg(reinterpret_cast<const float4*>(a.We_t + (size_t)d * H + lane * 4));
#pragma unroll
      for (int r = 0; r < 4; ++r) {
        float xv = hin[warp * 4 + r][d];
        acc[r][0] = fmaf(xv, w.x, acc[r][0]);
        acc[r][1] = fmaf(xv, w.y, acc[r][1]);
        acc[r][2] = fmaf(xv, w.z, acc[r][2]);
        acc[r][3] = fmaf(xv, w.w, acc[r][3]);
      }
    }
    const float4 bb = __ldg(reinterpret_cast<const float4*>(a.be + lane * 4));
#pragma unroll
    for (int r = 0; r < 4; ++r) {
      float4 o = make_float4(acc[r][0] + bb.x, acc[r][1] + bb.y, acc[r][2] + bb.z, acc[r][3] + bb.w);
      *reinterpret_cast<float4*>(hs + (warp * 4 + r) * LDX + lane * 4) = o;
      int g = g0 + warp * 4 + r;
      if (g < n_total) *reinterpret_cast<float4*>(a.h + (size_t)g * H + lane * 4) = o;
    }
  }
  __syncwarp();
  if (a.AB != nullptr) project_ab(hs + warp * 4 * LDX, a.proj, a.AB, a.ABmax, g0, n_total, warp, lane);
}

struct NodeArgs {
  float* h;
  const float* agg;
  const float* nm;
  const float* W3_t; const float* b3; const float* W4_t; const float* b4;
  ProjW proj1; float* AB1; float* ABmax1;
  ProjW proj2; float* AB2; float* ABmax2;
};

template <int ACT = ACT_SILU>
__global__ void __launch_bounds__(256) k_node(int n_total, NodeArgs a) {
  extern __shared__ __align__(16) float sm_node[];
  float* hs = sm_node;
  float* as = sm_node + NODE_TM * LDX;
  float* hid = as + NODE_TM * LDX;
  const int tid = threadIdx.x, lane = tid & 31, warp = tid >> 5;
  const int g0 = blockIdx.x * NODE_TM;
#pragma unroll
  for (int r = 0; r < 4; ++r) {
    int row = warp * 4 + r, g = g0 + row;
    float4 hv = make_float4(0, 0, 0, 0), av = hv;
    if (g < n_total) {
      hv = *reinterpret_cast<const float4*>(a.h + (size_t)g * H + lane * 4);
      av = *reinterpret_cast<const float4*>(a.agg + (size_t)g * H + lane * 4);
    }
    *reinterpret_cast<float4*>(hs + row * LDX + lane * 4) = hv;
    *reinterpret_cast<float4*>(as + row * LDX + lane * 4) = av;
  }
  __syncwarp();
  float acc[4][4];
  zero_acc(acc);
  warp_gemm_4x4<H>(hs + warp * 4 * LDX, a.W3_t, lane, acc);
  warp_gemm_4x4<H>(as + warp * 4 * LDX, a.W3_t + (size_t)H * H, lane, acc);
  {
    const float4 bb = __ldg(reinterpret_cast<const float4*>(a.b3 + lane * 4));
#pragma unroll
    for (int r = 0; r < 4; ++r)
      *reinterpret_cast<float4*>(hid + (warp * 4 + r) * LDX + lane * 4) =
          make_float4(act_f<ACT>(acc[r][0] + bb.x), act_f<ACT>(acc[r][1] + bb.y), act_f<ACT>(acc[r][2] + bb.z),
                      act_f<ACT>(acc[r][3] + bb.w));
  }
  __syncwarp();
  zero_acc(acc);
  warp_gemm_4x4<H>(hid + warp * 4 * LDX, a.W4_t, lane, acc);
  {
    const float4 bb = __ldg(reinterpret_cast<const float4*>(a.b4 + lane * 4));
#pragma unroll
    for (int r = 0; r < 4; ++r) {
      int row = warp * 4 + r, g = g0 + row;
      float m = g < n_total ? a.nm[g] : 0.f;
      float4 hv = *reinterpret_cast<const float4*>(hs + row * LDX + lane * 4);
      float4 o = make_float4((hv.x + (acc[r][0] + bb.x)) * m, (hv.y + (acc[r][1] + bb.y)) * m,
                             (hv.z + (acc[r][2] + bb.z)) * m, (hv.w + (acc[r][3] + bb.w)) * m);
      __syncwarp();
      *reinterpret_cast<float4*>(hs + row * LDX + lane * 4) = o;
      if (g < n_total) *reinterpret_cast<float4*>(a.h + (size_t)g * H + lane * 4) = o;
    }
  }
  __syncwarp();
  if (a.AB1 != nullptr) project_ab(hs + warp * 4 * LDX, a.proj1, a.AB1, a.ABmax1, g0, n_total, warp, lane);
  if (a.AB2 != nullptr) project_ab(hs + warp * 4 * LDX, a.proj2, a.AB2, a.ABmax2, g0, n_total, warp, lane);
}

__device__ __forceinline__ float edge_weight(int graph_type, const int8_t* __restrict__ em_mol, int N, int i, int j,
                                             int ci, int cj, float d0) {
  if (graph_type == 0) return em_mol != nullptr ? (float)em_mol[(size_t)i * N + j] : 1.0f;
  if (graph_type == 4)
    return ((em_mol == nullptr || em_mol[(size_t)i * N + j] != 0) && d0 < 6.0f) ? 1.f : 0.f;
  if (i == j || ci == 0 || cj == 0) return 0.f;
  float dist = sqrtf(d0);
  if (graph_type == 1) return dist <= 4.0f ? 1.f : 0.f;
  if (ci == 3 || cj == 3) return 0.f;
  if (ci == 1 && cj == 1) return 1.f;
  if (ci == 2 && cj == 2) return dist <= 4.0f ? 1.f : 0.f;
  float cut = graph_type == 2 ? 4.0f : 10.0f;
  return dist <= cut ? 1.f : 0.f;
}

constexpr int CUT_TN = 128;
constexpr int CUT_MAXR = 28;
constexpr int CUT_REC = 32;

__device__ __forceinline__ void cut_pack_rows(int b, int N, int nrows, const int* __restrict__ rowlist ,
                                              const int* degn, int* srt, int* row_bin, int* row_pos, int* row_start,
                                              int* bin_rem, int* bin_cnt, int* misc, int* __restrict__ recs,
                                              int* __restrict__ n_recs) {
  const int tid = threadIdx.x, lane = tid & 31, warp = tid >> 5;
  if (tid == 0) { misc[0] = 0; misc[1] = 0; }
  __syncthreads();
  for (int s = tid; s < nrows; s += blockDim.x) {
    const int node = rowlist[s], d = degn[node];
    if (d <= CUT_TN) {
      int rank = 0;
      for (int s2 = 0; s2 < nrows; ++s2) {
        const int d2 = degn[rowlist[s2]];
        rank += (d2 <= CUT_TN && (d2 > d || (d2 == d && s2 < s))) ? 1 : 0;
      }
      srt[rank] = node;
      atomicAdd(&misc[0], 1);
    } else {
      row_pos[node] = atomicAdd(&misc[1], 1);
    }
  }
  __syncthreads();
  const int n_light = misc[0], n_heavy = misc[1];
  if (warp == 0) {
    int nb = 0, first_open = 0;
    const int d_min = n_light > 0 ? degn[srt[n_light - 1]] : 0;
    for (int idx = 0; idx < n_light; ++idx) {
      const int node = srt[idx], d = degn[node];
      int found = -1;
      for (int base = first_open; base < nb && found < 0; base += 32) {
        const int bb = base + lane;
// ... 779 lines not shown
```

### difflinker_b200/csrc/kernels_tc.cuh

```cuda
#pragma once
#include <cuda_fp16.h>

#include <cmath>
#include <cstdio>
#include <type_traits>
#include <vector>

#include "../../include/difflinker_b200.h"
#include "kernels_simt.cuh"

namespace dl {
namespace tc {

constexpr bool AVAILABLE = true;
constexpr int TN = 128;
constexpr int MAXR = 32;
constexpr int KC = 16;
constexpr int W_LBO = H * 16;
constexpr int B_LBO = TN * 16 + 16;
constexpr int SBO = 128;
constexpr int W_BYTES = KC * W_LBO;
constexpr int B_BYTES = KC * B_LBO;
constexpr float F16_TARGET = 16384.0f;

constexpr int N_STAGE = 2;
constexpr int N_ACC = 4;

constexpr int W_EPI = 0;
constexpr int N_EPI_WARPS = 8;
constexpr int W_LOAD = 8;
constexpr int W_TBL = 9;
constexpr int N_TBL_WARPS = 3;
constexpr int W_PROD = 12;
constexpr int N_PROD_WARPS = 8;
constexpr int EDGE_TC_THREADS = 32 * (W_PROD + N_PROD_WARPS);
constexpr int REGS_EPI = 112, REGS_CTRL = 64;
constexpr int BAR_TURN0 = 3, BAR_TURN1 = 4;

constexpr int OFF_WHI = 0;
constexpr int OFF_WLO = OFF_WHI + W_BYTES;
constexpr int OFF_ST = OFF_WLO + W_BYTES;
constexpr int STAGE_BYTES = 2 * B_BYTES;
constexpr int OFF_TBL = OFF_ST + N_STAGE * STAGE_BYTES;
constexpr int TBL_HDR = 0;
constexpr int TBL_ROWOFF = 64;
constexpr int TBL_COLOFF = TBL_ROWOFF + TN * 4;
constexpr int TBL_D = TBL_COLOFF + TN * 4;
constexpr int TBL_D0 = TBL_D + TN * 4;
constexpr int TBL_SC = TBL_D0 + TN * 4;
constexpr int TBL_EM = TBL_SC + TN * 4;
constexpr int TBL_CD = TBL_EM + TN * 8;
constexpr int TBL_ROWNODE = TBL_CD + TN * 12;
constexpr int TBL_ROWSTART = TBL_ROWNODE + MAXR * 4;
constexpr int TBL_BYTES = TBL_ROWSTART + (MAXR + 4) * 4;
constexpr int OFF_B2W5 = OFF_TBL + N_ACC * TBL_BYTES;
constexpr int OFF_TX = OFF_B2W5 + H * 8;
constexpr int OFF_BAR = OFF_TX + TN * 12;
constexpr int BAR_W = 0, BAR_FULL = 8, BAR_EMPTY = BAR_FULL + 8 * N_STAGE, BAR_TBL = BAR_EMPTY + 8 * N_STAGE,
              BAR_TEMPTY = BAR_TBL + 8 * N_ACC, BAR_END = BAR_TEMPTY + 8 * N_ACC;
constexpr int SMEM_BYTES = OFF_BAR + BAR_END + 1024;
static_assert(SMEM_BYTES <= 232448, "k_edge_tc exceeds the 227 KB of shared memory a CTA can opt into");
static_assert(TBL_BYTES % 16 == 0, "table slots must keep 16-byte alignment");

__device__ __forceinline__ uint32_t smem_u32(const void* p) { return (uint32_t)__cvta_generic_to_shared(p); }

__device__ __forceinline__ void mbar_init(uint32_t bar, uint32_t count) {
  asm volatile("mbarrier.init.shared::cta.b64 [%0], %1;" ::"r"(bar), "r"(count));
}
__device__ __forceinline__ void mbar_expect_tx(uint32_t bar, uint32_t bytes) {
  asm volatile("mbarrier.arrive.expect_tx.shared::cta.b64 _, [%0], %1;" ::"r"(bar), "r"(bytes) : "memory");
}
__device__ __constant__ int c_wait_mode = 1;
constexpr uint32_t WAIT_HINT_NS = 20000;
__device__ __forceinline__ void mbar_wait(uint32_t bar, uint32_t parity) {
  uint32_t done = 0;
  const int mode = c_wait_mode;
  if (mode == 1) {
    for (uint32_t spin = 0; spin < (1u << 20); ++spin) {
      asm volatile(
          "{\n\t.reg .pred p;\n\t"
          "mbarrier.try_wait.parity.shared::cta.b64 p, [%1], %2, %3;\n\t"
          "selp.u32 %0, 1, 0, p;\n\t}"
          : "=r"(done)
          : "r"(bar), "r"(parity), "r"(WAIT_HINT_NS)
          : "memory");
      if (done) return;
    }
    __trap();
  }
  for (uint32_t spin = 0; spin < (1u << 28); ++spin) {
    asm volatile(
        "{\n\t.reg .pred p;\n\t"
        "mbarrier.try_wait.parity.shared::cta.b64 p, [%1], %2;\n\t"
        "selp.u32 %0, 1, 0, p;\n\t}"
        : "=r"(done)
        : "r"(bar), "r"(parity)
        : "memory");
    if (done) return;
    if (mode == 2) __nanosleep(32);
  }
  __trap();
}
__device__ __forceinline__ void mbar_arrive(uint32_t bar) {
  asm volatile("mbarrier.arrive.shared::cta.b64 _, [%0];" ::"r"(bar) : "memory");
}
__device__ __forceinline__ void named_sync(int id, int nthreads) {
  asm volatile("bar.sync %0, %1;" ::"r"(id), "r"(nthreads) : "memory");
}
__device__ __forceinline__ void named_arrive(int id, int nthreads) {
  asm volatile("bar.arrive %0, %1;" ::"r"(id), "r"(nthreads) : "memory");
}
__device__ __forceinline__ void mbar_wait_relaxed(uint32_t bar, uint32_t parity) {
  uint32_t done = 0;
  for (uint32_t spin = 0; spin < (1u << 24); ++spin) {
    asm volatile(
        "{\n\t.reg .pred p;\n\t"
        "mbarrier.try_wait.parity.shared::cta.b64 p, [%1], %2;\n\t"
        "selp.u32 %0, 1, 0, p;\n\t}"
        : "=r"(done)
        : "r"(bar), "r"(parity)
        : "memory");
    if (done) return;
    __nanosleep(64);
  }
  __trap();
}
__device__ __forceinline__ void fence_barrier_init() { asm volatile("fence.mbarrier_init.release.cluster;" ::: "memory"); }
__device__ __forceinline__ void fence_proxy_async() { asm volatile("fence.proxy.async.shared::cta;" ::: "memory"); }

__device__ __forceinline__ void bulk_g2s(uint32_t dst, const void* src, uint32_t bytes, uint32_t bar) {
  asm volatile("cp.async.bulk.shared::cluster.global.mbarrier::complete_tx::bytes [%0], [%1], %2, [%3];" ::"r"(dst),
               "l"(src), "r"(bytes), "r"(bar)
               : "memory");
}

__device__ __forceinline__ uint64_t wg_desc(uint32_t saddr, uint32_t lbo, uint32_t sbo) {
  return (uint64_t)((saddr & 0x3FFFFu) >> 4) | ((uint64_t)(lbo >> 4) << 16) | ((uint64_t)(sbo >> 4) << 32);
}
__device__ __forceinline__ void wg_fence() { asm volatile("wgmma.fence.sync.aligned;" ::: "memory"); }
__device__ __forceinline__ void wg_commit() { asm volatile("wgmma.commit_group.sync.aligned;" ::: "memory"); }
__device__ __forceinline__ void wg_wait_all() { asm volatile("wgmma.wait_group.sync.aligned 0;" ::: "memory"); }
__device__ __forceinline__ void fence_acc(float (&d)[64]) {
#pragma unroll
  for (int i = 0; i < 64; ++i) asm volatile("" : "+f"(d[i])::"memory");
}
template <int TRANS_B>
__device__ __forceinline__ void wgmma_m64n128k16(float (&d)[64], uint64_t adesc, uint64_t bdesc, uint32_t accumulate) {
  asm volatile(
      "{\n\t.reg .pred p;\n\t"
      "setp.ne.b32 p, %66, 0;\n\t"
      "wgmma.mma_async.sync.aligned.m64n128k16.f32.f16.f16 "
      "{%0, %1, %2, %3, %4, %5, %6, %7, %8, %9, %10, %11, %12, %13, %14, %15, %16, %17, %18, %19, %20, %21, %22, %23, %24, %25, %26, %27, %28, %29, %30, %31, %32, %33, %34, %35, %36, %37, %38, %39, %40, %41, %42, %43, %44, %45, %46, %47, %48, %49, %50, %51, %52, %53, %54, %55, %56, %57, %58, %59, %60, %61, %62, %63}, %64, %65, p, 1, 1, 0, %67;\n\t}"
      : "+f"(d[0]), "+f"(d[1]), "+f"(d[2]), "+f"(d[3]), "+f"(d[4]), "+f"(d[5]), "+f"(d[6]), "+f"(d[7]), "+f"(d[8]), "+f"(d[9]), "+f"(d[10]), "+f"(d[11]), "+f"(d[12]), "+f"(d[13]), "+f"(d[14]), "+f"(d[15]), "+f"(d[16]), "+f"(d[17]), "+f"(d[18]), "+f"(d[19]), "+f"(d[20]), "+f"(d[21]), "+f"(d[22]), "+f"(d[23]), "+f"(d[24]), "+f"(d[25]), "+f"(d[26]), "+f"(d[27]), "+f"(d[28]), "+f"(d[29]), "+f"(d[30]), "+f"(d[31]), "+f"(d[32]), "+f"(d[33]), "+f"(d[34]), "+f"(d[35]), "+f"(d[36]), "+f"(d[37]), "+f"(d[38]), "+f"(d[39]), "+f"(d[40]), "+f"(d[41]), "+f"(d[42]), "+f"(d[43]), "+f"(d[44]), "+f"(d[45]), "+f"(d[46]), "+f"(d[47]), "+f"(d[48]), "+f"(d[49]), "+f"(d[50]), "+f"(d[51]), "+f"(d[52]), "+f"(d[53]), "+f"(d[54]), "+f"(d[55]), "+f"(d[56]), "+f"(d[57]), "+f"(d[58]), "+f"(d[59]), "+f"(d[60]), "+f"(d[61]), "+f"(d[62]), "+f"(d[63])
      : "l"(adesc), "l"(bdesc), "r"(accumulate), "n"(TRANS_B));
}
template <int TRANS_B = 0>
__device__ __forceinline__ void mma_3xf16(float (&d)[64], uint32_t a_hi, uint32_t a_lo, uint32_t a_lbo, uint32_t b_hi,
                                          uint32_t b_lo, uint32_t b_lbo, uint32_t b_ks_stride, int nks, bool accumulate) {
#pragma unroll
  for (int ks = 0; ks < nks; ++ks) {
    const uint64_t ah = wg_desc(a_hi + ks * 2 * a_lbo, a_lbo, SBO), al = wg_desc(a_lo + ks * 2 * a_lbo, a_lbo, SBO);
    const uint64_t bh = wg_desc(b_hi + ks * b_ks_stride, b_lbo, SBO), bl = wg_desc(b_lo + ks * b_ks_stride, b_lbo, SBO);
    wgmma_m64n128k16<TRANS_B>(d, al, bh, (accumulate || ks > 0) ? 1u : 0u);
    wgmma_m64n128k16<TRANS_B>(d, ah, bl, 1u);
    wgmma_m64n128k16<TRANS_B>(d, ah, bh, 1u);
  }
}
template <int TRANS_B = 0>
__device__ __forceinline__ void gemm_3xf16(float (&d)[64], uint32_t a_hi, uint32_t a_lo, uint32_t a_lbo, uint32_t b_hi,
                                           uint32_t b_lo, uint32_t b_lbo, uint32_t b_ks_stride, int nks, bool accumulate) {
  fence_acc(d);
  wg_fence();
  mma_3xf16<TRANS_B>(d, a_hi, a_lo, a_lbo, b_hi, b_lo, b_lbo, b_ks_stride, nks, accumulate);
  wg_commit();
  wg_wait_all();
  fence_acc(d);
}

__device__ __forceinline__ void split2v(float2 v, uint32_t& hi, uint32_t& lo) {
  __half2 h = __float22half2_rn(v);
  float2 back = __half22float2(h);
  __half2 l = __float22half2_rn(fadd2(v, make_float2(-back.x, -back.y)));
  hi = *reinterpret_cast<uint32_t*>(&h);
  lo = *reinterpret_cast<uint32_t*>(&l);
}
__device__ __forceinline__ void split2(float a, float b, uint32_t& hi, uint32_t& lo) {
  __half2 h = __floats2half2_rn(a, b);
  float2 back = __half22float2(h);
  __half2 l = __floats2half2_rn(a - back.x, b - back.y);
  hi = *reinterpret_cast<uint32_t*>(&h);
  lo = *reinterpret_cast<uint32_t*>(&l);
}
__device__ __forceinline__ int gcl_row_of_edge(int e) { return 8 * ((e & 31) >> 1) + 2 * (e >> 5) + (e & 1); }
struct Tile {
  int b, nc, slot0, nrt, c0, ncc;
  bool first_chunk, last_chunk;
  const int* rows;
  int Et;
  int start;
  int node;
};

template <bool COORD>
struct TileIter {
  const int4* list;
  const int* rowlist;
  int N, wi_end, wi, rt, c0, cache_base, lane;
  int4 cache;
  __device__ TileIter(const Plan& p, int N_) : N(N_), rt(0), c0(0), cache_base(-(1 << 30)), lane(threadIdx.x & 31) {
    list = COORD ? p.xitems : p.items;
    rowlist = COORD ? p.xrowidx : p.rowidx;
    const int total = COORD ? *p.n_xitems : *p.n_items;
    const int per = total / (int)gridDim.x, extra = total % (int)gridDim.x, c = (int)blockIdx.x;
    wi = c * per + min(c, extra);
    wi_end = wi + per + (c < extra ? 1 : 0);
    cache = make_int4(0, 0, 0, 0);
  }
  __device__ bool next(Tile& t) {
    while (wi < wi_end) {
      if (wi - cache_base >= 32) {
        cache_base = wi;
        cache = list[min(wi + lane, wi_end - 1)];
      }
      const int src = wi - cache_base;
      const int b = __shfl_sync(0xffffffffu, cache.x, src), r_begin = __shfl_sync(0xffffffffu, cache.y, src);
      const int r_count = __shfl_sync(0xffffffffu, cache.z, src), nc = __shfl_sync(0xffffffffu, cache.w, src);
      int per = nc >= TN ? 1 : TN / max(nc, 1);
      if (per > MAXR) per = MAXR;
      if (rt >= r_count || nc <= 0) { wi += 1; rt = 0; c0 = 0; continue; }
      t.b = b; t.nc = nc; t.slot0 = r_begin + rt; t.nrt = min(per, r_count - rt);
      t.c0 = c0; t.ncc = min(TN, nc - c0);
      t.first_chunk = c0 == 0; t.last_chunk = c0 + TN >= nc;
      t.rows = rowlist + (size_t)b * N;
      c0 += TN;
      if (c0 >= nc) { c0 = 0; rt += per; }
      return true;
    }
    return false;
  }
};

struct RecIter {
  const int* recs;
  int n, k, G, lane, cur, nxt, chunk;
  __device__ RecIter(const int* recs_, const int* n_recs) : recs(recs_), lane(threadIdx.x & 31), cur(0), chunk(0) {
    n = *n_recs; G = (int)gridDim.x; k = (int)blockIdx.x;
    nxt = k < n ? recs[(size_t)k * CUT_REC + lane] : 0;
  }
  __device__ bool next(Tile& t) {
    if (chunk == 0) {
      if (k >= n) return false;
      cur = nxt;
      const int kn = k + G;
      nxt = kn < n ? recs[(size_t)kn * CUT_REC + lane] : 0;
    }
    const int w1 = __shfl_sync(0xffffffffu, cur, 1), v2 = __shfl_sync(0xffffffffu, cur, 2);
    const int info = __shfl_sync(0xffffffffu, cur, (4 + lane) & 31);
    t.b = __shfl_sync(0xffffffffu, cur, 0);
    t.nc = 0; t.slot0 = 0; t.rows = nullptr;
    if (((w1 >> 8) & 1) == 0) {
      t.nrt = w1 & 0xff; t.Et = v2; t.ncc = v2; t.c0 = 0; t.first_chunk = true; t.last_chunk = true;
      t.node = info & 0xffff; t.start = info >> 16;
      k += G;
    } else {
      const int deg = v2, c0 = chunk * TN;
      t.nrt = 1; t.Et = min(TN, deg - c0); t.ncc = t.Et; t.c0 = c0;
      t.first_chunk = chunk == 0; t.last_chunk = c0 + TN >= deg;
      t.node = __shfl_sync(0xffffffffu, cur, 4) & 0xffff;
      t.start = lane == 0 ? 0 : t.Et;
      ++chunk;
      if (t.last_chunk) { chunk = 0; k += G; }
    }
    return true;
  }
};

template <bool COORD, bool SPARSE>
__device__ __forceinline__ typename std::conditional<SPARSE, RecIter, TileIter<COORD>>::type make_iter(const EdgeArgs& a, int N) {
  if constexpr (SPARSE) return RecIter(a.recs, a.n_recs);
  else return TileIter<COORD>(a.plan, N);
}

template <bool COORD, bool SPARSE = false, int OPT = 0>
__global__ void __launch_bounds__(EDGE_TC_THREADS, 1) k_edge_tc(Geom gm, EdgeArgs a, const __half* __restrict__ w2tc) {
  constexpr bool MEAN = (OPT & OPT_MEAN) != 0, TANH = (OPT & OPT_TANH) != 0, EMB = (OPT & OPT_SIN) != 0;
  static_assert(COORD || !TANH, "tanh only bounds the coordinate update");
  extern __shared__ uint8_t smem_raw[];
  uint8_t* sm = smem_raw + ((1024u - (smem_u32(smem_raw) & 1023u)) & 1023u);
  const uint32_t sbase = smem_u32(sm);
  const int tid = threadIdx.x, lane = tid & 31, warp = tid >> 5;
  const int N = gm.N;

  const uint32_t bars = sbase + OFF_BAR;
  float2* b2w5 = reinterpret_cast<float2*>(sm + OFF_B2W5);

  if (tid == 0) {
    mbar_init(bars + BAR_W, 1);
    for (int i = 0; i < N_STAGE; ++i) { mbar_init(bars + BAR_FULL + 8 * i, N_PROD_WARPS); mbar_init(bars + BAR_EMPTY + 8 * i, N_EPI_WARPS); }
    for (int i = 0; i < N_ACC; ++i) {
      mbar_init(bars + BAR_TBL + 8 * i, 1);
      mbar_init(bars + BAR_TEMPTY + 8 * i, N_EPI_WARPS);
    }
    fence_barrier_init();
  }
  if (tid < H) b2w5[tid] = make_float2(a.b2[tid], COORD ? a.w5[tid] : 0.f);
  __syncthreads();

  if (warp >= W_LOAD && warp < W_PROD) {
    asm volatile("setmaxnreg.dec.sync.aligned.u32 %0;" ::"n"(REGS_CTRL));
  if (warp >= W_TBL && warp < W_TBL + N_TBL_WARPS) {
    const int tw = warp - W_TBL;
    typename std::conditional<SPARSE, RecIter, TileIter<COORD>>::type iter = make_iter<COORD, SPARSE>(a, N);
    Tile cur;
    for (int t = 0;; ++t) {
      const int acc = t & (N_ACC - 1);
      const bool more = iter.next(cur);
      if (t % N_TBL_WARPS != tw) { if (!more) break; continue; }
      if (t >= N_ACC) mbar_wait_relaxed(bars + BAR_TEMPTY + 8 * acc, ((t - N_ACC) / N_ACC) & 1);
      uint8_t* tb = sm + OFF_TBL + acc * TBL_BYTES;
      int* hdr = reinterpret_cast<int*>(tb + TBL_HDR);
      if (more) {
        const int Et = SPARSE ? cur.Et : cur.nrt * cur.ncc;
        const size_t gb = (size_t)cur.b * N;
        int heavy_deg = 0;
        if constexpr (MEAN && SPARSE) {
          const int w1 = __shfl_sync(0xffffffffu, iter.cur, 1), v2 = __shfl_sync(0xffffffffu, iter.cur, 2);
          heavy_deg = ((w1 >> 8) & 1) ? v2 : 0;
        }
        if (lane == 0) {
          hdr[0] = Et; hdr[1] = cur.nrt; hdr[2] = cur.ncc;
          hdr[3] = (cur.first_chunk ? 1 : 0) | (cur.last_chunk ? 2 : 0);
          hdr[4] = cur.b;
          if (MEAN && SPARSE) hdr[6] = heavy_deg;
        }
        if (SPARSE) {
          if (lane < cur.nrt) {
            reinterpret_cast<int*>(tb + TBL_ROWNODE)[lane] = cur.node;
            reinterpret_cast<int*>(tb + TBL_ROWSTART)[lane] = cur.start;
          }
          if (lane == 0) reinterpret_cast<int*>(tb + TBL_ROWSTART)[cur.nrt] = Et;
        } else {
          if (lane < cur.nrt) {
            reinterpret_cast<int*>(tb + TBL_ROWNODE)[lane] = cur.rows[cur.slot0 + lane];
            reinterpret_cast<int*>(tb + TBL_ROWSTART)[lane] = lane * cur.ncc;
          }
          if (lane == 0) reinterpret_cast<int*>(tb + TBL_ROWSTART)[cur.nrt] = Et;
        }
        bool any_rescale = false;
#pragma unroll
        for (int e = lane; e < TN; e += 32) {
          const int ev = min(e, Et - 1);
          int i, j;
          float ew_list = 1.f;
          if (SPARSE) {
            int rr = 0;
            for (int r = 1; r < cur.nrt; ++r) rr += ev >= __shfl_sync(0xffffffffu, cur.start, r) ? 1 : 0;
            i = __shfl_sync(0xffffffffu, cur.node, rr);
            const int first_col = __shfl_sync(0xffffffffu, cur.start, rr);
            const int raw = a.nbr[(gb + i) * N + cur.c0 + (ev - first_col)];
            j = raw & 0x7fffffff;
            ew_list = raw < 0 ? 0.f : 1.f;
          } else {
            const int rr = ev / cur.ncc, jj = ev - rr * cur.ncc;
            i = cur.rows[cur.slot0 + rr];
            j = a.plan.colidx[gb + cur.c0 + jj];
          }
          const float4 xi = a.x4[gb + i], xj = a.x4[gb + j], yi = a.x04[gb + i], yj = a.x04[gb + j];
          const float dx = xi.x - xj.x, dy = xi.y - xj.y, dz = xi.z - xj.z;
          const float ex = yi.x - yj.x, ey = yi.y - yj.y, ez = yi.z - yj.z;
          float d, d0;
          if constexpr (EMB) {
            d = radial_rn(dx, dy, dz); d0 = radial_rn(ex, ey, ez);
          } else {
            d = dx * dx + dy * dy + dz * dz;
            d0 = ex * ex + ey * ey + ez * ez;
          }
          int ci = 0, cj = 0;
          if (!SPARSE && gm.graph_type != 0) { ci = a.cls[gb + i]; cj = a.cls[gb + j]; }
          reinterpret_cast<int*>(tb + TBL_ROWOFF)[e] = (int)((gb + i) * 2 * H);
          reinterpret_cast<int*>(tb + TBL_COLOFF)[e] = (int)((gb + j) * 2 * H + H);
          reinterpret_cast<float*>(tb + TBL_D)[e] = d;
          reinterpret_cast<float*>(tb + TBL_D0)[e] = d0;
          const float bound = EMB ? a.ABmax[(gb + i) * 2] + a.ABmax[(gb + j) * 2 + 1] + a.wdmax
                                  : a.ABmax[(gb + i) * 2] + a.ABmax[(gb + j) * 2 + 1] + d * a.wdmax + d0 * a.w0max;
          float sc = 1.0f;
          if (!(bound <= F16_TARGET)) {
            const int ex2 = ((__float_as_int(bound) >> 23) & 0xff) - 127;
            sc = __int_as_float(max(127 + 13 - ex2, 1) << 23);
          }
          reinterpret_cast<float*>(tb + TBL_SC)[e] = sc;
          any_rescale |= (sc != 1.0f);
          const float ew = SPARSE ? ew_list
                                  : edge_weight(gm.graph_type, a.edge_mask ? a.edge_mask + gb * N : nullptr, N, i, j, ci, cj, d0);
          reinterpret_cast<float2*>(tb + TBL_EM)[e] =
              COORD ? make_float2(ew, a.w2_descale / sc)
                    : make_float2(ew * -0.6931471805599453f, (a.w2_descale / sc) * -1.4426950408889634f);
          if (COORD) {
            const float inv = 1.0f / (sqrtf(d + 1e-8f) + gm.norm_constant);
            float* cds = reinterpret_cast<float*>(tb + TBL_CD);
            cds[e * 3 + 0] = dx * inv; cds[e * 3 + 1] = dy * inv; cds[e * 3 + 2] = dz * inv;
          }
        }
        any_rescale = __any_sync(0xffffffffu, any_rescale);
        if (lane == 0) hdr[5] = any_rescale ? 1 : 0;
      } else if (lane == 0) {
        hdr[0] = 0;
      }
      __syncwarp();
      if (lane == 0) mbar_arrive(bars + BAR_TBL + 8 * acc);
      if (!more) break;
    }
  } else if (warp == W_LOAD) {
    if (lane == 0) {
      mbar_expect_tx(bars + BAR_W, 2 * W_BYTES);
      bulk_g2s(sbase + OFF_WHI, w2tc, 2 * W_BYTES, bars + BAR_W);
    }
  }
  } else if (warp >= W_PROD) {
    const int pw = warp - W_PROD;
    const int kc = lane & 15, esub = lane >> 4;
    float2 wdr[4], w0r[4];
#pragma unroll
    for (int q = 0; q < 4; ++q) {
      wdr[q] = make_float2(__ldg(a.wd + kc * 8 + 2 * q), __ldg(a.wd + kc * 8 + 2 * q + 1));
      w0r[q] = make_float2(__ldg(a.w0 + kc * 8 + 2 * q), __ldg(a.w0 + kc * 8 + 2 * q + 1));
    }
    for (int t = 0;; ++t) {
      const int acc = t & (N_ACC - 1), s = t & (N_STAGE - 1);
      mbar_wait(bars + BAR_TBL + 8 * acc, (t / N_ACC) & 1);
      const uint8_t* tb = sm + OFF_TBL + acc * TBL_BYTES;
      const int Et = reinterpret_cast<const int*>(tb + TBL_HDR)[0];
      if (t >= N_STAGE) mbar_wait(bars + BAR_EMPTY + 8 * s, ((t - N_STAGE) / N_STAGE) & 1);
      if (Et > 0) {
        const int* rowoff = reinterpret_cast<const int*>(tb + TBL_ROWOFF);
        const int* coloff = reinterpret_cast<const int*>(tb + TBL_COLOFF);
        const float* dv = reinterpret_cast<const float*>(tb + TBL_D);
        const float* d0v = reinterpret_cast<const float*>(tb + TBL_D0);
        const float* scv = reinterpret_cast<const float*>(tb + TBL_SC);
        uint8_t* bhi = sm + OFF_ST + s * STAGE_BYTES + kc * B_LBO;
        uint8_t* blo = bhi + B_BYTES;
        const bool rescale = reinterpret_cast<const int*>(tb + TBL_HDR)[5] != 0;
        constexpr int ITEMS = TN / (2 * N_PROD_WARPS);
        float4 pa0, pa1, pb[2][2];
        const int e_base = ITEMS * (2 * pw + esub);
        int ro_cur = rowoff[e_base];
        {
          const float* ap = a.AB + ro_cur + kc * 8;
          pa0 = __ldg(reinterpret_cast<const float4*>(ap)); pa1 = __ldg(reinterpret_cast<const float4*>(ap + 4));
        }
#pragma unroll
        for (int pf = 0; pf < 2; ++pf) {
          const float* bp = a.AB + coloff[e_base + pf] + kc * 8;
          pb[pf][0] = __ldg(reinterpret_cast<const float4*>(bp)); pb[pf][1] = __ldg(reinterpret_cast<const float4*>(bp + 4));
        }
#pragma unroll
        for (int it = 0; it < ITEMS; ++it) {
          const int e = e_base + it;
          const int slot = it & 1;
          const float4 b0 = pb[slot][0], b1 = pb[slot][1];
          if (it + 2 < ITEMS) {
            const float* bp = a.AB + coloff[e + 2] + kc * 8;
            pb[slot][0] = __ldg(reinterpret_cast<const float4*>(bp)); pb[slot][1] = __ldg(reinterpret_cast<const float4*>(bp + 4));
          }
          const int ro = rowoff[e];
          if (ro != ro_cur) {
            ro_cur = ro;
            const float* ap = a.AB + ro + kc * 8;
            pa0 = __ldg(reinterpret_cast<const float4*>(ap)); pa1 = __ldg(reinterpret_cast<const float4*>(ap + 4));
          }
          const float4 a0 = pa0, a1 = pa1;
          float2 pre_emb[4];
          if constexpr (EMB) {
            const int kf = kc < 12 ? kc : kc - 12;
            float sn, cs;
            sincosf(sin_arg(kf < N_SIN_FREQ ? dv[e] : d0v[e], kf % N_SIN_FREQ), &sn, &cs);
            pre_emb[0] = fadd2(make_float2(a0.x, a0.y), make_float2(b0.x, b0.y));
            pre_emb[1] = fadd2(make_float2(a0.z, a0.w), make_float2(b0.z, b0.w));
            pre_emb[2] = fadd2(make_float2(a1.x, a1.y), make_float2(b1.x, b1.y));
            pre_emb[3] = fadd2(make_float2(a1.z, a1.w), make_float2(b1.z, b1.w));
#pragma unroll 2
            for (int k = 0; k < N_SIN_FEAT; ++k) {
              const int src = (k / 12) * N_SIN_FREQ + k % N_SIN_FREQ;
              const float ev = __shfl_sync(0xffffffffu, (k % 12) < N_SIN_FREQ ? sn : cs, src, 16);
              const float4 w0 = __ldg(reinterpret_cast<const float4*>(a.we + k * H + kc * 8));
              const float4 w1 = __ldg(reinterpret_cast<const float4*>(a.we + k * H + kc * 8 + 4));
              const float2 ee = make_float2(ev, ev);
              pre_emb[0] = ffma2(ee, make_float2(w0.x, w0.y), pre_emb[0]);
              pre_emb[1] = ffma2(ee, make_float2(w0.z, w0.w), pre_emb[1]);
              pre_emb[2] = ffma2(ee, make_float2(w1.x, w1.y), pre_emb[2]);
              pre_emb[3] = ffma2(ee, make_float2(w1.z, w1.w), pre_emb[3]);
            }
          }
          if (e < Et) {
            float2 sv[4];
            if constexpr (EMB) {
#pragma unroll
              for (int q = 0; q < 4; ++q) sv[q] = usig2(pre_emb[q]);
            } else {
              const float d = dv[e], d0 = d0v[e];
              const float2 dd = make_float2(d, d), dd0 = make_float2(d0, d0);
              const float2 av[4] = {make_float2(a0.x, a0.y), make_float2(a0.z, a0.w), make_float2(a1.x, a1.y), make_float2(a1.z, a1.w)};
              const float2 bv[4] = {make_float2(b0.x, b0.y), make_float2(b0.z, b0.w), make_float2(b1.x, b1.y), make_float2(b1.z, b1.w)};
  #pragma unroll
              for (int q = 0; q < 4; ++q)
                sv[q] = usig2(ffma2(dd0, w0r[q], ffma2(dd, wdr[q], fadd2(av[q], bv[q]))));
            }
            if (rescale) {
              const float sc = scv[e];
#pragma unroll
              for (int q = 0; q < 4; ++q) sv[q] = fmul2(sv[q], make_float2(sc, sc));
            }
            uint4 hi, lo;
            split2v(sv[0], hi.x, lo.x); split2v(sv[1], hi.y, lo.y);
            split2v(sv[2], hi.z, lo.z); split2v(sv[3], hi.w, lo.w);
            const int row = COORD ? e : gcl_row_of_edge(e);
            *reinterpret_cast<uint4*>(bhi + row * 16) = hi;
            *reinterpret_cast<uint4*>(blo + row * 16) = lo;
          }
        }
        fence_proxy_async();
      }
      __syncwarp();
      if (lane == 0) mbar_arrive(bars + BAR_FULL + 8 * s);
      if (Et <= 0) break;
    }
  } else {
    asm volatile("setmaxnreg.inc.sync.aligned.u32 %0;" ::"n"(REGS_EPI));
    const int g = warp >> 2;
    const int wq = warp & 3, q = lane & 3;
    const int r0 = 64 * g + 16 * wq + (lane >> 2);
    float* txs = reinterpret_cast<float*>(sm + OFF_TX);
    float2 run = make_float2(0.f, 0.f);
    float run3 = 0.f;
    float d[64];
#pragma unroll
    for (int i = 0; i < 64; ++i) d[i] = 0.f;
    mbar_wait(bars + BAR_W, 0);
    for (int t = 0;; ++t) {
      const int acc = t & (N_ACC - 1), s = t & (N_STAGE - 1);
      if (!COORD && g == 0 && t > 0) named_sync(BAR_TURN0, 32 * N_EPI_WARPS);
      mbar_wait(bars + BAR_TBL + 8 * acc, (t / N_ACC) & 1);
      const uint8_t* tb = sm + OFF_TBL + acc * TBL_BYTES;
      const int* hdr = reinterpret_cast<const int*>(tb + TBL_HDR);
      const int Et = hdr[0];
      if (Et <= 0) break;
      const uint32_t bhi = sbase + OFF_ST + s * STAGE_BYTES, blo = bhi + B_BYTES;
      if (!COORD) {
        if (g == 1) named_sync(BAR_TURN1, 32 * N_EPI_WARPS);
        mbar_wait(bars + BAR_FULL + 8 * s, (t / N_STAGE) & 1);
        fence_acc(d);
        wg_fence();
        mma_3xf16(d, sbase + OFF_WHI + g * 1024, sbase + OFF_WLO + g * 1024, W_LBO, bhi, blo, B_LBO, 2 * B_LBO, 8, false);
        wg_commit();
        named_arrive(g == 0 ? BAR_TURN1 : BAR_TURN0, 32 * N_EPI_WARPS);
        wg_wait_all();
        fence_acc(d);
      } else {
        mbar_wait(bars + BAR_FULL + 8 * s, (t / N_STAGE) & 1);
        gemm_3xf16(d, bhi + g * 1024, blo + g * 1024, B_LBO, sbase + OFF_WHI, sbase + OFF_WLO, W_LBO, 2 * W_LBO, 8, false);
      }
      __syncwarp();
      if (lane == 0) mbar_arrive(bars + BAR_EMPTY + 8 * s);

      const int nrt = hdr[1];
      const bool first_chunk = hdr[3] & 1, last_chunk = hdr[3] & 2;
      const size_t gb = (size_t)hdr[4] * N;
      const float2* emds = reinterpret_cast<const float2*>(tb + TBL_EM);
      const int* rownode = reinterpret_cast<const int*>(tb + TBL_ROWNODE);
      const int* rowstart = reinterpret_cast<const int*>(tb + TBL_ROWSTART);
      if (!COORD) {
        const float2 bias = make_float2(b2w5[r0].x * -1.4426950408889634f, b2w5[r0 + 8].x * -1.4426950408889634f);
        const float inv_norm = 1.0f / gm.normalization_factor;
        const float inv_n = 1.0f / (float)N;
        auto put = [&](int r, float2 v) {
          float* dst = a.agg + (gb + rownode[r]) * H;
          if constexpr (MEAN) {
            const float inv = SPARSE ? rcp_approx((float)(hdr[6] > 0 ? hdr[6] : rowstart[r + 1] - rowstart[r])) : inv_n;
            dst[r0] = v.x * inv; dst[r0 + 8] = v.y * inv;
          } else {
            dst[r0] = v.x * inv_norm; dst[r0 + 8] = v.y * inv_norm;
          }
        };
        const int E0 = 32 * q;
        const bool has = E0 < Et;
        int cur = 0;
        if (has) { while (rowstart[cur + 1] <= E0) ++cur; }
        const int hrow = cur;
        uint32_t bmask = 0;
        int nr = cur + 1;
        if (has) { for (; nr <= nrt && rowstart[nr] < E0 + 32; ++nr) bmask |= 1u << (rowstart[nr] - E0); }
        const bool open_end = has && nr <= nrt && rowstart[nr] > E0 + 32;
        const bool cut = Et < E0 + 32;
        const uint32_t wmask = __reduce_or_sync(0xffffffffu, bmask);
        float2 hsum = make_float2(0.f, 0.f), sum = make_float2(0.f, 0.f);
        bool in_head = true;
#pragma unroll
        for (int tt = 0; tt < 32; ++tt) {
          if (wmask & (1u << tt)) {
            const bool here = (bmask >> tt) & 1u;
            if (here && !in_head) put(cur, sum);
            hsum = here && in_head ? sum : hsum;
            sum = here ? make_float2(0.f, 0.f) : sum;
            in_head = in_head && !here;
            cur += here ? 1 : 0;
          }
          const float2 ed = emds[E0 + tt];
          const float2 u = ffma2(make_float2(d[(tt >> 1) * 4 + (tt & 1)], d[(tt >> 1) * 4 + 2 + (tt & 1)]),
                                 make_float2(ed.y, ed.y), bias);
          const float2 v = fmul2(usig2(u), make_float2(ed.x, ed.x));
          sum = fadd2(sum, v);
        }
        if (in_head) hsum = sum;
        const float2 lsum = sum;
        const bool cont_in = has && rowstart[hrow] < E0;
        float2 cin = (q == 0 && nrt == 1 && !first_chunk) ? run : make_float2(0.f, 0.f);
#pragma unroll
        for (int k = 0; k < 3; ++k) {
          const float2 cout = in_head ? fadd2(cin, hsum) : lsum;
          const float px = __shfl_up_sync(0xffffffffu, cout.x, 1, 4), py = __shfl_up_sync(0xffffffffu, cout.y, 1, 4);
          if (q == k + 1 && cont_in) cin = make_float2(px, py);
        }
        const float2 htot = fadd2(cin, hsum);
        if (nrt == 1) {
          const int src = (lane & ~3) | ((Et - 1) >> 5);
          run = make_float2(__shfl_sync(0xffffffffu, htot.x, src), __shfl_sync(0xffffffffu, htot.y, src));
        }
        if (has && last_chunk) {
          if (!in_head || !open_end) put(hrow, htot);
          if (!in_head && !open_end && !cut) put(cur, lsum);
        }
        __syncwarp();
        if (lane == 0) mbar_arrive(bars + BAR_TEMPTY + 8 * acc);
      } else {
        const float2 eda = emds[min(r0, Et - 1)], edb = emds[min(r0 + 8, Et - 1)];
        float2 pa = make_float2(0.f, 0.f), pb = make_float2(0.f, 0.f);
#pragma unroll
        for (int j = 0; j < 16; ++j) {
          const float2 w0 = b2w5[8 * j + 2 * q], w1 = b2w5[8 * j + 2 * q + 1];
          const float2 va = ffma2(make_float2(d[4 * j], d[4 * j + 1]), make_float2(eda.y, eda.y), make_float2(w0.x, w1.x));
          const float2 vb = ffma2(make_float2(d[4 * j + 2], d[4 * j + 3]), make_float2(edb.y, edb.y), make_float2(w0.x, w1.x));
          pa = ffma2(silu2(va), make_float2(w0.y, w1.y), pa);
          pb = ffma2(silu2(vb), make_float2(w0.y, w1.y), pb);
        }
        float phia = pa.x + pa.y, phib = pb.x + pb.y;
        phia += __shfl_xor_sync(0xffffffffu, phia, 1); phib += __shfl_xor_sync(0xffffffffu, phib, 1);
        phia += __shfl_xor_sync(0xffffffffu, phia, 2); phib += __shfl_xor_sync(0xffffffffu, phib, 2);
        const float* cds = reinterpret_cast<const float*>(tb + TBL_CD);
        if constexpr (TANH) {
          const float range = a.coords_range;
          if (q == 0 && r0 < Et) {
            const float th = tanhf(phia);
#pragma unroll
            for (int k = 0; k < 3; ++k) txs[r0 * 3 + k] = cds[r0 * 3 + k] * th * range * eda.x;
          }
          if (q == 0 && r0 + 8 < Et) {
            const int e = r0 + 8;
            const float th = tanhf(phib);
#pragma unroll
            for (int k = 0; k < 3; ++k) txs[e * 3 + k] = cds[e * 3 + k] * th * range * edb.x;
          }
        } else {
          if (q == 0 && r0 < Et) {
            const float w = phia * eda.x;
            txs[r0 * 3 + 0] = cds[r0 * 3 + 0] * w; txs[r0 * 3 + 1] = cds[r0 * 3 + 1] * w; txs[r0 * 3 + 2] = cds[r0 * 3 + 2] * w;
          }
          if (q == 0 && r0 + 8 < Et) {
            const int e = r0 + 8;
            const float w = phib * edb.x;
            txs[e * 3 + 0] = cds[e * 3 + 0] * w; txs[e * 3 + 1] = cds[e * 3 + 1] * w; txs[e * 3 + 2] = cds[e * 3 + 2] * w;
          }
        }
        named_sync(2, 32 * N_EPI_WARPS);
        if (tid < nrt * 3) {
          const int rr = tid / 3, dim = tid - rr * 3;
          float sacc = (nrt == 1 && !first_chunk) ? run3 : 0.f;
          const int col0 = rowstart[rr];
          const int ncc = rowstart[rr + 1] - col0;
          for (int jj = 0; jj < ncc; ++jj) sacc += txs[(col0 + jj) * 3 + dim];
          if (nrt == 1) run3 = sacc;
          if (last_chunk) {
            const int i = rownode[rr];
            const float lm = a.linker_mask ? a.linker_mask[gb + i] : 1.f;
            const float xv = a.x[(gb + i) * 3 + dim];
            float div = gm.normalization_factor;
            if constexpr (MEAN) div = SPARSE ? (float)(hdr[6] > 0 ? hdr[6] : ncc) : (float)N;
            const float xn = (xv + (sacc / div) * lm) * a.nm[gb + i];
            a.x_out[(gb + i) * 3 + dim] = xn;
            reinterpret_cast<float*>(a.x4_out + gb + i)[dim] = xn;
          }
        }
        named_sync(2, 32 * N_EPI_WARPS);
        if (lane == 0) mbar_arrive(bars + BAR_TEMPTY + 8 * acc);
      }
    }
  }
}

template <typename K>
inline bool opt_in_smem(K kern) {
  return cudaFuncSetAttribute(kern, cudaFuncAttributeMaxDynamicSharedMemorySize, SMEM_BYTES) == cudaSuccess;
}
constexpr int OPT_ALL = OPT_TANH | OPT_MEAN | OPT_SIN;
template <bool COORD, bool SPARSE, int OPT = 0>
inline bool opt_in_all() {
  if constexpr (OPT > OPT_ALL) {
    return true;
  } else {
    if constexpr (COORD || !(OPT & OPT_TANH))
      if (!opt_in_smem(k_edge_tc<COORD, SPARSE, OPT>)) return false;
    return opt_in_all<COORD, SPARSE, OPT + 1>();
  }
}
inline dl_status configure() {
  const bool ok = opt_in_all<true, false>() && opt_in_all<true, true>() && opt_in_all<false, false>() && opt_in_all<false, true>();
  return ok ? DL_OK : DL_ERR_CUDA;
}

constexpr double NEG_LN2 = -0.6931471805599453094;
constexpr double NEG_LOG2E = -1.4426950408889634074;

inline size_t pack_w2(const std::vector<float>& W_in, std::vector<__half>& blob, float* descale) {
  std::vector<float> W(W_in.size());
  for (size_t i = 0; i < W.size(); ++i) W[i] = (float)((double)W_in[i] * NEG_LN2);
  while (blob.size() % 64) blob.push_back(__float2half(0.f));
  const size_t off = blob.size();
  blob.resize(off + 2 * (size_t)KC * H * 8);
  float mx = 0.f;
  for (float v : W) mx = std::max(mx, std::fabs(v));
  int ex = 0;
  if (mx > 0.f && std::isfinite(mx)) { std::frexp(mx, &ex); ex -= 1; }
  const int sh = std::min(std::max(13 - ex, -40), 40);
  const float scale = std::ldexp(1.0f, sh);
  *descale = std::ldexp(1.0f, -sh);
  for (int kc = 0; kc < KC; ++kc)
    for (int c = 0; c < H; ++c)
      for (int u = 0; u < 8; ++u) {
        const float v = W[(size_t)c * H + kc * 8 + u] * scale;
        const __half hi = __float2half_rn(v);
        const __half lo = __float2half_rn(v - __half2float(hi));
        blob[off + ((size_t)kc * H + c) * 8 + u] = hi;
        blob[off + (size_t)KC * H * 8 + ((size_t)kc * H + c) * 8 + u] = lo;
      }
  return off;
}

template <bool COORD, bool SPARSE, int OPT = 0>
inline void launch_opt(int opt, const Geom& gm, const EdgeArgs& ea, const __half* w, int num_sms, cudaStream_t st) {
  if constexpr (OPT <= OPT_ALL) {
    if constexpr (COORD || !(OPT & OPT_TANH))
      if (opt == OPT) { k_edge_tc<COORD, SPARSE, OPT><<<num_sms, EDGE_TC_THREADS, SMEM_BYTES, st>>>(gm, ea, w); return; }
    launch_opt<COORD, SPARSE, OPT + 1>(opt, gm, ea, w, num_sms, st);
  }
}

inline dl_status launch_edge_tc(const Geom& gm, const EdgeArgs& ea, bool coord, int opt, const void* w2_tc, int num_sms,
                                cudaStream_t st) {
  if (!coord && (opt & OPT_TANH)) return DL_ERR_INVALID;
  if (ea.recs == nullptr && gm.graph_type != 0 && (opt & OPT_MEAN)) return DL_ERR_INVALID;
  const __half* w = reinterpret_cast<const __half*>(w2_tc);
  if (ea.recs != nullptr) {
    if (coord) launch_opt<true, true>(opt, gm, ea, w, num_sms, st);
    else launch_opt<false, true>(opt, gm, ea, w, num_sms, st);
  } else if (coord) launch_opt<true, false>(opt, gm, ea, w, num_sms, st);
  else launch_opt<false, false>(opt, gm, ea, w, num_sms, st);
  return DL_OK;
}

constexpr int PN = 256;
constexpr int P_LBO = PN * 16 + 16;
constexpr int P_OFF_BHI = 2 * W_BYTES, P_OFF_BLO = P_OFF_BHI + KC * P_LBO;
constexpr int P_SMEM_BYTES = P_OFF_BLO + KC * P_LBO + 1024;
template <bool B_MN>
__global__ void __launch_bounds__(256, 1) k_wgmma_probe(const __half* __restrict__ A ,
                                                        const __half* __restrict__ Bm ,
                                                        float* __restrict__ D ) {
  extern __shared__ uint8_t smem_raw[];
  uint8_t* sm = smem_raw + ((1024u - (smem_u32(smem_raw) & 1023u)) & 1023u);
  const uint32_t sbase = smem_u32(sm);
  const int tid = threadIdx.x, lane = tid & 31, warp = tid >> 5;
  for (int idx = tid; idx < 2 * KC * H; idx += 256) {
    const int copy = idx / (KC * H), rem = idx % (KC * H), kcx = rem / H, row = rem % H;
    *reinterpret_cast<uint4*>(sm + (copy ? OFF_WLO : OFF_WHI) + kcx * W_LBO + row * 16) =
        *reinterpret_cast<const uint4*>(A + (size_t)idx * 8);
  }
  constexpr int MN_LBO = (PN / 8) * 128;
  for (int idx = tid; idx < 2 * KC * PN; idx += 256) {
    const int copy = idx / (KC * PN), rem = idx % (KC * PN), kcx = rem / PN, row = rem % PN;
    if (!B_MN) {
      *reinterpret_cast<uint4*>(sm + (copy ? P_OFF_BLO : P_OFF_BHI) + kcx * P_LBO + row * 16) =
          *reinterpret_cast<const uint4*>(Bm + (size_t)idx * 8);
    } else {
      for (int u = 0; u < 8; ++u)
        *reinterpret_cast<__half*>(sm + (copy ? P_OFF_BLO : P_OFF_BHI) + kcx * MN_LBO + (row >> 3) * 128 + u * 16 + (row & 7) * 2) =
            Bm[(size_t)idx * 8 + u];
    }
  }
  fence_proxy_async();
  __syncthreads();
  const int g = warp >> 2;
  const int r0 = 64 * g + 16 * (warp & 3) + (lane >> 2), q = lane & 3;
  float d[64];
  for (int nh = 0; nh < 2; ++nh) {
    const uint32_t bhi = sbase + P_OFF_BHI + nh * (B_MN ? 16 * 128 : 128 * 16), blo = bhi + (P_OFF_BLO - P_OFF_BHI);
    if (B_MN)
      gemm_3xf16<1>(d, sbase + OFF_WHI + g * 1024, sbase + OFF_WLO + g * 1024, W_LBO, bhi, blo, MN_LBO, 2 * MN_LBO, 8, false);
    else
      gemm_3xf16<0>(d, sbase + OFF_WHI + g * 1024, sbase + OFF_WLO + g * 1024, W_LBO, bhi, blo, P_LBO, 2 * P_LBO, 8, false);
#pragma unroll
    for (int j = 0; j < 16; ++j) {
      const int col = nh * 128 + 8 * j + 2 * q;
      D[(size_t)r0 * PN + col] = d[4 * j]; D[(size_t)r0 * PN + col + 1] = d[4 * j + 1];
      D[(size_t)(r0 + 8) * PN + col] = d[4 * j + 2]; D[(size_t)(r0 + 8) * PN + col + 1] = d[4 * j + 3];
    }
  }
}

inline dl_status selftest(int , float* max_abs_err, float* max_rel_err, bool b_mn_major = false) {
  std::vector<float> A((size_t)H * H), Bv((size_t)PN * H);
  uint32_t s = 12345u;
  auto rnd = [&]() { s = s * 1664525u + 1013904223u; return ((s >> 8) & 0xFFFF) / 65536.0f - 0.5f; };
  for (auto& v : A) v = rnd() * 0.2f;
  for (auto& v : Bv) v = rnd() * 3.0f;
  auto pack = [&](const std::vector<float>& M, int rows) {
    std::vector<__half> out(2 * (size_t)KC * rows * 8);
    for (int kc = 0; kc < KC; ++kc)
      for (int r = 0; r < rows; ++r)
        for (int u = 0; u < 8; ++u) {
          const float v = M[(size_t)r * H + kc * 8 + u];
          const __half hi = __float2half_rn(v);
          out[((size_t)kc * rows + r) * 8 + u] = hi;
          out[(size_t)KC * rows * 8 + ((size_t)kc * rows + r) * 8 + u] = __float2half_rn(v - __half2float(hi));
        }
    return out;
  };
  std::vector<__half> Ap = pack(A, H), Bp = pack(Bv, PN);
  __half *dA = nullptr, *dB = nullptr;
  float* dD = nullptr;
  if (cudaMalloc(&dA, Ap.size() * 2) != cudaSuccess || cudaMalloc(&dB, Bp.size() * 2) != cudaSuccess ||
      cudaMalloc(&dD, (size_t)H * PN * 4) != cudaSuccess)
    return DL_ERR_CUDA;
  cudaMemcpy(dA, Ap.data(), Ap.size() * 2, cudaMemcpyHostToDevice);
  cudaMemcpy(dB, Bp.data(), Bp.size() * 2, cudaMemcpyHostToDevice);
  cudaMemset(dD, 0, (size_t)H * PN * 4);
  if (b_mn_major) {
    cudaFuncSetAttribute(k_wgmma_probe<true>, cudaFuncAttributeMaxDynamicSharedMemorySize, P_SMEM_BYTES);
    k_wgmma_probe<true><<<1, 256, P_SMEM_BYTES>>>(dA, dB, dD);
  } else {
    cudaFuncSetAttribute(k_wgmma_probe<false>, cudaFuncAttributeMaxDynamicSharedMemorySize, P_SMEM_BYTES);
    k_wgmma_probe<false><<<1, 256, P_SMEM_BYTES>>>(dA, dB, dD);
  }
  cudaError_t err = cudaDeviceSynchronize();
  std::vector<float> D((size_t)H * PN);
  cudaMemcpy(D.data(), dD, D.size() * 4, cudaMemcpyDeviceToHost);
  cudaFree(dA); cudaFree(dB); cudaFree(dD);
  if (err != cudaSuccess) {
    fprintf(stderr, "[dl selftest] k_wgmma_probe failed: %s\n", cudaGetErrorString(err));
    return DL_ERR_CUDA;
  }
  double ma = 0, mr = 0, mref = 0;
  for (int m = 0; m < H; ++m)
    for (int n = 0; n < PN; ++n) {
      double ref = 0;
      for (int k = 0; k < H; ++k) ref += (double)A[(size_t)m * H + k] * (double)Bv[(size_t)n * H + k];
      ma = std::max(ma, std::fabs(ref - (double)D[(size_t)m * PN + n]));
      mref = std::max(mref, std::fabs(ref));
    }
  mr = ma / std::max(mref, 1e-30);
  if (max_abs_err) *max_abs_err = (float)ma;
  if (max_rel_err) *max_rel_err = (float)mr;
  fprintf(stderr, "[dl selftest] 3xFP16 wgmma 128x256x128 (B %s-major): max abs err %.3e (rel to max |ref| %.3e)\n",
          b_mn_major ? "MN" : "K", ma, mr);
  return DL_OK;
}

}
}
```

Before: 191.0.

## Pipeline coordinate-update epilogue with double-buffered tx and dense load-balanced iteration

Restructures the coordinate edge kernel in several ways. Dense work items become one row each, and the plan builder balances them across SMs by edge count. A new DenseIter packs partial rows into full tiles with a carry across chunks. The per-row reduction moves from an all-epilogue named barrier into a separate consumer warp fed by double-buffered tx slots with mbarriers, and the MMA path now shares the async wgmma turn-taking used by the non-coord path. It also folds the separate x copy kernel into the last node kernel launch. The aim is to remove epilogue stalls, load imbalance and one launch per layer, at the cost of extra shared memory and more complex synchronisation that could be wrong.

```diff
diff --git a/difflinker_b200/csrc/common.cuh b/difflinker_b200/csrc/common.cuh
--- a/difflinker_b200/csrc/common.cuh
+++ b/difflinker_b200/csrc/common.cuh
@@ -127,6 +127,7 @@
   const int* n_xmols;
   const int4* xitems;
   const int* n_xitems;
+  const int* xcta_begin;
 };
 
 struct Geom {
diff --git a/difflinker_b200/csrc/dl_engine.cu b/difflinker_b200/csrc/dl_engine.cu
--- a/difflinker_b200/csrc/dl_engine.cu
+++ b/difflinker_b200/csrc/dl_engine.cu
@@ -47,7 +47,7 @@
   int *nbr = nullptr, *recs = nullptr, *xrecs = nullptr, *n_recs = nullptr;
   float4 *x04 = nullptr, *xa4 = nullptr, *xb4 = nullptr;
   int *rowidx = nullptr, *colidx = nullptr, *xrowidx = nullptr, *nr = nullptr, *nc = nullptr, *nxr = nullptr,
-      *n_items = nullptr, *xmols = nullptr, *n_xmols = nullptr, *n_xitems = nullptr;
+      *n_items = nullptr, *xmols = nullptr, *n_xmols = nullptr, *n_xitems = nullptr, *xcta_begin = nullptr;
   int4* items = nullptr;
   int4* xitems = nullptr;
   int* tile_ctr = nullptr;
@@ -304,6 +304,7 @@
   WSA(agg, n * H); WSA(z, n * xd); WSA(eps, n * xd); WSA(cls, n); WSA(x04, n); WSA(xa4, n); WSA(xb4, n); WSA(ABgmax, n * 2); WSA(ABcmax, n * 2);
   WSA(rowidx, n); WSA(colidx, n); WSA(xrowidx, n); WSA(nr, B); WSA(nc, B); WSA(nxr, B); WSA(n_items, 1);
   WSA(xmols, B); WSA(n_xmols, 1); WSA(items, n); WSA(xitems, n); WSA(n_xitems, 1); WSA(tile_ctr, 64); WSA(seeds, B);
+  if (e->use_tc) WSA(xcta_begin, e->num_sms + 1);
   if (e->use_tc && e->cfg.graph_type != 0) { WSA(nbr, n * N); WSA(recs, n * CUT_REC); WSA(xrecs, n * CUT_REC); WSA(n_recs, 2); }
 #undef WSA
   ws.B = B; ws.N = N;
@@ -314,7 +315,7 @@
   Plan p;
   p.rowidx = ws.rowidx; p.colidx = ws.colidx; p.xrowidx = ws.xrowidx; p.nr = ws.nr; p.nc = ws.nc; p.nxr = ws.nxr;
   p.items = ws.items; p.n_items = ws.n_items; p.xmols = ws.xmols; p.n_xmols = ws.n_xmols;
-  p.xitems = ws.xitems; p.n_xitems = ws.n_xitems;
+  p.xitems = ws.xitems; p.n_xitems = ws.n_xitems; p.xcta_begin = ws.xcta_begin;
   return p;
 }
 
@@ -338,7 +339,7 @@
 constexpr int PLAN_MAX_N = 48 * 1024 / (2 * (int)sizeof(int));
 
 dl_status build_plan(Workspace& ws, int B, int N, int graph_type, const int8_t* node_mask, const float* linker_mask,
-                     const int8_t* edge_mask, int tile_edges, int max_rows, cudaStream_t st) {
+                     const int8_t* edge_mask, int tile_edges, int max_rows, cudaStream_t st, int n_cta = 0) {
   if (N > PLAN_MAX_N) {
     set_err("N = %d exceeds the work plan's limit of %d rows per molecule", N, PLAN_MAX_N);
     return DL_ERR_UNSUPPORTED;
@@ -348,7 +349,7 @@
                                                   ws.colidx, ws.xrowidx, ws.nr, ws.nc, ws.nxr);
   LAUNCH_CHECK();
   k_plan_items<<<1, 1, 0, st>>>(B, tile_edges, max_rows, 1, max_rows, ws.nr, ws.nc, ws.nxr, ws.items, ws.n_items, ws.xmols,
-                                ws.n_xmols, ws.xitems, ws.n_xitems);
+                                ws.n_xmols, ws.xitems, ws.n_xitems, n_cta, ws.xcta_begin);
   LAUNCH_CHECK();
   return DL_OK;
 }
@@ -356,7 +357,7 @@
 dl_status build_forward_plan(dl_engine* e, int B, int N, const int8_t* node_mask, const float* linker_mask,
                              const int8_t* edge_mask, cudaStream_t st) {
   const dl_status s = build_plan(e->ws, B, N, e->cfg.graph_type, node_mask, linker_mask, edge_mask,
-                                 e->use_tc ? tc::TN : ET, e->use_tc ? tc::MAXR : MAXR, st);
+                                 e->use_tc ? tc::TN : ET, e->use_tc ? tc::MAXR : MAXR, st, e->use_tc ? e->num_sms : 0);
   if (s == DL_OK) e->launches += 2;
   return s;
 }
@@ -516,7 +517,8 @@
       if (st2 != DL_OK) return st2;
 
       if (e->use_tc) {
-        const tcn::NodeTcArgs ta = node_tc_args(e, w, l, s);
+        tcn::NodeTcArgs ta = node_tc_args(e, w, l, s);
+        if (s + 1 == S) { ta.x = xin; ta.x_next = xout; ta.x4 = xin4; ta.x4_next = xout4; }
         TIMED(ta.n_proj == 2 ? "k_node_tc(2 proj)" : "k_node_tc(1 proj)", st, (tcn::launch_node(n, ta, st)));
       } else {
         NodeArgs na{};
@@ -530,9 +532,11 @@
       LAUNCH_CHECK();
       e->launches += 1;
     }
-    k_copy_x<<<(n * 3 + 255) / 256, 256, 0, st>>>(n * 3, xin, xout, e->use_tc ? xin4 : nullptr, xout4);
-    LAUNCH_CHECK();
-    e->launches += 1;
+    if (!e->use_tc) {
+      k_copy_x<<<(n * 3 + 255) / 256, 256, 0, st>>>(n * 3, xin, xout, nullptr, nullptr);
+      LAUNCH_CHECK();
+      e->launches += 1;
+    }
     const EqW& w = e->eq[l];
     const EdgeArgs ea = edge_args(e, w, true, io.edge_mask, io.linker_mask, xin, xin4, xout, xout4, w.w5);
     e->times.begin(st, "edge COORD");
diff --git a/difflinker_b200/csrc/kernels_node_tc.cuh b/difflinker_b200/csrc/kernels_node_tc.cuh
--- a/difflinker_b200/csrc/kernels_node_tc.cuh
+++ b/difflinker_b200/csrc/kernels_node_tc.cuh
@@ -38,6 +38,8 @@
   float p_descale[2];
   float* AB[2];
   float* ABmax[2];
+  const float* x; float* x_next;
+  const float4* x4; float4* x4_next;
 };
 
 __device__ __forceinline__ float pow2_scale_for(float bound) {
@@ -106,6 +108,10 @@
   chain_wait();
   if (tid == 0) chain_release();
   if (tid < TM) nms[tid] = tid < n_live ? a.nm[g0 + tid] : 0.f;
+  if (a.x_next != nullptr) {
+    for (int k = tid; k < 3 * n_live; k += 32 * NW) a.x_next[(size_t)g0 * 3 + k] = a.x[(size_t)g0 * 3 + k];
+    for (int k = tid; k < n_live; k += 32 * NW) a.x4_next[g0 + k] = a.x4[g0 + k];
+  }
 
   const int g = warp >> 2, q = lane & 3;
   const int c0 = 64 * g + 16 * (warp & 3) + (lane >> 2);
diff --git a/difflinker_b200/csrc/kernels_simt.cuh b/difflinker_b200/csrc/kernels_simt.cuh
--- a/difflinker_b200/csrc/kernels_simt.cuh
+++ b/difflinker_b200/csrc/kernels_simt.cuh
@@ -53,7 +53,7 @@
                              const int* __restrict__ nc, const int* __restrict__ nxr, int4* __restrict__ items,
                              int* __restrict__ n_items, int* __restrict__ xmols, int* __restrict__ n_xmols,
                              int4* __restrict__ xitems, int* __restrict__ n_xitems, int n_cta = 0,
-                             int* __restrict__ cta_begin = nullptr, int* __restrict__ xcta_begin = nullptr) {
+                             int* __restrict__ xcta_begin = nullptr) {
   if (threadIdx.x != 0 || blockIdx.x != 0) return;
   int cnt = 0, xc = 0, xi = 0;
   for (int b = 0; b < B; ++b) {
@@ -66,38 +66,23 @@
     }
     if (nxr[b] > 0 && c > 0) {
       xmols[xc++] = b;
-      int per;
-      if (col_pad > 1) {
-        const int cp = (c + col_pad - 1) / col_pad * col_pad;
-        per = cp >= tile_edges ? 1 : tile_edges / cp;
-        if (per > max_rows_gcl) per = max_rows_gcl;
-      } else {
-        per = c >= tile_edges ? 1 : tile_edges / c;
-        if (per > max_rows) per = max_rows;
-      }
-      for (int r0 = 0; r0 < nxr[b]; r0 += per) xitems[xi++] = make_int4(b, r0, min(per, nxr[b] - r0), c);
+      for (int r0 = 0; r0 < nxr[b]; ++r0) xitems[xi++] = make_int4(b, r0, 1, c);
     }
   }
   *n_items = cnt;
   *n_xmols = xc;
   *n_xitems = xi;
-  if (n_cta > 0 && cta_begin != nullptr) {
-    for (int pass = 0; pass < 2; ++pass) {
-      const int4* list = pass == 0 ? items : xitems;
-      const int total = pass == 0 ? cnt : xi;
-      int* out = pass == 0 ? cta_begin : xcta_begin;
-      if (out == nullptr) continue;
-      long long sum = 0;
-      for (int k = 0; k < total; ++k) sum += (long long)list[k].z * ((list[k].w + col_pad - 1) / col_pad * col_pad) + 32;
-      long long run = 0;
-      int c = 0;
-      out[0] = 0;
-      for (int k = 0; k < total; ++k) {
-        while (c + 1 < n_cta && run * n_cta >= (long long)(c + 1) * sum) out[++c] = k;
-        run += (long long)list[k].z * ((list[k].w + col_pad - 1) / col_pad * col_pad) + 32;
-      }
-      while (c < n_cta) out[++c] = total;
-    }
+  if (n_cta > 0 && xcta_begin != nullptr) {
+    long long sum = 0;
+    for (int k = 0; k < xi; ++k) sum += xitems[k].w;
+    long long run = 0;
+    int c = 0;
+    xcta_begin[0] = 0;
+    for (int k = 0; k < xi; ++k) {
+      while (c + 1 < n_cta && run * n_cta >= (long long)(c + 1) * sum) xcta_begin[++c] = k;
+      run += xitems[k].w;
+    }
+    while (c < n_cta) xcta_begin[++c] = xi;
   }
 }
 
diff --git a/difflinker_b200/csrc/kernels_tc.cuh b/difflinker_b200/csrc/kernels_tc.cuh
--- a/difflinker_b200/csrc/kernels_tc.cuh
+++ b/difflinker_b200/csrc/kernels_tc.cuh
@@ -54,10 +54,13 @@
 constexpr int TBL_ROWSTART = TBL_ROWNODE + MAXR * 4;
 constexpr int TBL_BYTES = TBL_ROWSTART + (MAXR + 4) * 4;
 constexpr int OFF_B2W5 = OFF_TBL + N_ACC * TBL_BYTES;
+constexpr int N_TX = 2;
 constexpr int OFF_TX = OFF_B2W5 + H * 8;
-constexpr int OFF_BAR = OFF_TX + TN * 12;
+constexpr int OFF_CARRY = OFF_TX + N_TX * TN * 12;
+constexpr int OFF_BAR = OFF_CARRY + 32;
 constexpr int BAR_W = 0, BAR_FULL = 8, BAR_EMPTY = BAR_FULL + 8 * N_STAGE, BAR_TBL = BAR_EMPTY + 8 * N_STAGE,
-              BAR_TEMPTY = BAR_TBL + 8 * N_ACC, BAR_END = BAR_TEMPTY + 8 * N_ACC;
+              BAR_TEMPTY = BAR_TBL + 8 * N_ACC, BAR_TXFULL = BAR_TEMPTY + 8 * N_ACC, BAR_TXEMPTY = BAR_TXFULL + 8 * N_TX,
+              BAR_END = BAR_TXEMPTY + 8 * N_TX;
 constexpr int SMEM_BYTES = OFF_BAR + BAR_END + 1024;
 static_assert(SMEM_BYTES <= 232448, "k_edge_tc exceeds the 227 KB of shared memory a CTA can opt into");
 static_assert(TBL_BYTES % 16 == 0, "table slots must keep 16-byte alignment");
@@ -199,18 +202,18 @@
   int Et;
   int start;
   int node;
+  int gbr, col;
 };
 
-template <bool COORD>
 struct TileIter {
   const int4* list;
   const int* rowlist;
   int N, wi_end, wi, rt, c0, cache_base, lane;
   int4 cache;
   __device__ TileIter(const Plan& p, int N_) : N(N_), rt(0), c0(0), cache_base(-(1 << 30)), lane(threadIdx.x & 31) {
-    list = COORD ? p.xitems : p.items;
-    rowlist = COORD ? p.xrowidx : p.rowidx;
-    const int total = COORD ? *p.n_xitems : *p.n_items;
+    list = p.items;
+    rowlist = p.rowidx;
+    const int total = *p.n_items;
     const int per = total / (int)gridDim.x, extra = total % (int)gridDim.x, c = (int)blockIdx.x;
     wi = c * per + min(c, extra);
     wi_end = wi + per + (c < extra ? 1 : 0);
@@ -240,6 +243,46 @@
   }
 };
 
+struct DenseIter {
+  const int4* list;
+  int N, wi, wi_end, pos, cache_base, lane;
+  int4 cache;
+  __device__ DenseIter(const Plan& p, int N_) : N(N_), pos(0), cache_base(-(1 << 30)), lane(threadIdx.x & 31) {
+    list = p.xitems;
+    wi = p.xcta_begin[blockIdx.x];
+    wi_end = p.xcta_begin[blockIdx.x + 1];
+    cache = make_int4(0, 0, 0, 0);
+  }
+  __device__ bool next(Tile& t) {
+    int Et = 0, nrt = 0;
+    t.first_chunk = true;
+    t.last_chunk = true;
+    while (wi < wi_end && Et < TN && nrt < MAXR) {
+      if (wi - cache_base >= 32) {
+        cache_base = wi;
+        cache = list[min(wi + lane, wi_end - 1)];
+      }
+      const int src = wi - cache_base;
+      const int b = __shfl_sync(0xffffffffu, cache.x, src), r0 = __shfl_sync(0xffffffffu, cache.y, src);
+      const int nxr = __shfl_sync(0xffffffffu, cache.z, src);
+      const int nc = __shfl_sync(0xffffffffu, cache.w, src);
+      if (nxr <= 0 || nc <= 0) { wi += 1; pos = 0; continue; }
+      const int r = pos / nc, col = pos - r * nc;
+      const int take = min(nc - col, TN - Et);
+      if (nrt == 0) t.first_chunk = col == 0;
+      t.last_chunk = col + take == nc;
+      if (lane == nrt) { t.start = Et; t.node = r0 + r; t.gbr = b * N; t.col = col; }
+      ++nrt;
+      Et += take;
+      pos += take;
+      if (pos == nxr * nc) { wi += 1; pos = 0; }
+    }
+    if (lane == nrt) t.start = Et;
+    t.nrt = nrt; t.Et = Et; t.ncc = Et; t.c0 = 0; t.b = 0; t.nc = 0; t.slot0 = 0; t.rows = nullptr;
+    return nrt > 0;
+  }
+};
+
 struct RecIter {
   const int* recs;
   int n, k, G, lane, cur, nxt, chunk;
@@ -276,14 +319,17 @@
 };
 
 template <bool COORD, bool SPARSE>
-__device__ __forceinline__ typename std::conditional<SPARSE, RecIter, TileIter<COORD>>::type make_iter(const EdgeArgs& a, int N) {
+using IterOf = typename std::conditional<SPARSE, RecIter, typename std::conditional<COORD, DenseIter, TileIter>::type>::type;
+template <bool COORD, bool SPARSE>
+__device__ __forceinline__ IterOf<COORD, SPARSE> make_iter(const EdgeArgs& a, int N) {
   if constexpr (SPARSE) return RecIter(a.recs, a.n_recs);
-  else return TileIter<COORD>(a.plan, N);
+  else return IterOf<COORD, SPARSE>(a.plan, N);
 }
 
 template <bool COORD, bool SPARSE = false, int OPT = 0>
 __global__ void __launch_bounds__(EDGE_TC_THREADS, 1) k_edge_tc(Geom gm, EdgeArgs a, const __half* __restrict__ w2tc) {
   constexpr bool MEAN = (OPT & OPT_MEAN) != 0, TANH = (OPT & OPT_TANH) != 0, EMB = (OPT & OPT_SIN) != 0;
+  constexpr bool DENSE = COORD && !SPARSE;
   static_assert(COORD || !TANH, "tanh only bounds the coordinate update");
   extern __shared__ uint8_t smem_raw[];
   uint8_t* sm = smem_raw + ((1024u - (smem_u32(smem_raw) & 1023u)) & 1023u);
@@ -299,8 +345,9 @@
     for (int i = 0; i < N_STAGE; ++i) { mbar_init(bars + BAR_FULL + 8 * i, N_PROD_WARPS); mbar_init(bars + BAR_EMPTY + 8 * i, N_EPI_WARPS); }
     for (int i = 0; i < N_ACC; ++i) {
       mbar_init(bars + BAR_TBL + 8 * i, 1);
-      mbar_init(bars + BAR_TEMPTY + 8 * i, N_EPI_WARPS);
-    }
+      mbar_init(bars + BAR_TEMPTY + 8 * i, COORD ? 1 : N_EPI_WARPS);
+    }
+    for (int i = 0; i < N_TX; ++i) { mbar_init(bars + BAR_TXFULL + 8 * i, N_EPI_WARPS); mbar_init(bars + BAR_TXEMPTY + 8 * i, 1); }
     fence_barrier_init();
   }
   if (tid < H) b2w5[tid] = make_float2(a.b2[tid], COORD ? a.w5[tid] : 0.f);
@@ -310,7 +357,7 @@
     asm volatile("setmaxnreg.dec.sync.aligned.u32 %0;" ::"n"(REGS_CTRL));
   if (warp >= W_TBL && warp < W_TBL + N_TBL_WARPS) {
     const int tw = warp - W_TBL;
-    typename std::conditional<SPARSE, RecIter, TileIter<COORD>>::type iter = make_iter<COORD, SPARSE>(a, N);
+    IterOf<COORD, SPARSE> iter = make_iter<COORD, SPARSE>(a, N);
     Tile cur;
     for (int t = 0;; ++t) {
       const int acc = t & (N_ACC - 1);
@@ -320,7 +367,7 @@
       uint8_t* tb = sm + OFF_TBL + acc * TBL_BYTES;
       int* hdr = reinterpret_cast<int*>(tb + TBL_HDR);
       if (more) {
-        const int Et = SPARSE ? cur.Et : cur.nrt * cur.ncc;
+        const int Et = (SPARSE || DENSE) ? cur.Et : cur.nrt * cur.ncc;
         const size_t gb = (size_t)cur.b * N;
         int heavy_deg = 0;
         if constexpr (MEAN && SPARSE) {
@@ -333,9 +380,17 @@
           hdr[4] = cur.b;
           if (MEAN && SPARSE) hdr[6] = heavy_deg;
         }
+        int row_i = 0;
         if (SPARSE) {
           if (lane < cur.nrt) {
             reinterpret_cast<int*>(tb + TBL_ROWNODE)[lane] = cur.node;
+            reinterpret_cast<int*>(tb + TBL_ROWSTART)[lane] = cur.start;
+          }
+          if (lane == 0) reinterpret_cast<int*>(tb + TBL_ROWSTART)[cur.nrt] = Et;
+        } else if (DENSE) {
+          if (lane < cur.nrt) {
+            row_i = a.plan.xrowidx[cur.gbr + cur.node];
+            reinterpret_cast<int*>(tb + TBL_ROWNODE)[lane] = cur.gbr + row_i;
             reinterpret_cast<int*>(tb + TBL_ROWSTART)[lane] = cur.start;
           }
           if (lane == 0) reinterpret_cast<int*>(tb + TBL_ROWSTART)[cur.nrt] = Et;
@@ -351,8 +406,17 @@
         for (int e = lane; e < TN; e += 32) {
           const int ev = min(e, Et - 1);
           int i, j;
+          size_t ge = gb;
           float ew_list = 1.f;
-          if (SPARSE) {
+          if constexpr (DENSE) {
+            int rr = 0;
+            for (int r = 1; r < cur.nrt; ++r) rr += ev >= __shfl_sync(0xffffffffu, cur.start, r) ? 1 : 0;
+            const int gbr = __shfl_sync(0xffffffffu, cur.gbr, rr);
+            i = __shfl_sync(0xffffffffu, row_i, rr);
+            const int jj = __shfl_sync(0xffffffffu, cur.col, rr) + ev - __shfl_sync(0xffffffffu, cur.start, rr);
+            ge = (size_t)gbr;
+            j = a.plan.colidx[ge + jj];
+          } else if (SPARSE) {
             int rr = 0;
             for (int r = 1; r < cur.nrt; ++r) rr += ev >= __shfl_sync(0xffffffffu, cur.start, r) ? 1 : 0;
             i = __shfl_sync(0xffffffffu, cur.node, rr);
@@ -365,7 +429,7 @@
             i = cur.rows[cur.slot0 + rr];
             j = a.plan.colidx[gb + cur.c0 + jj];
           }
-          const float4 xi = a.x4[gb + i], xj = a.x4[gb + j], yi = a.x04[gb + i], yj = a.x04[gb + j];
+          const float4 xi = a.x4[ge + i], xj = a.x4[ge + j], yi = a.x04[ge + i], yj = a.x04[ge + j];
           const float dx = xi.x - xj.x, dy = xi.y - xj.y, dz = xi.z - xj.z;
           const float ex = yi.x - yj.x, ey = yi.y - yj.y, ez = yi.z - yj.z;
           float d, d0;
@@ -376,13 +440,13 @@
             d0 = ex * ex + ey * ey + ez * ez;
           }
           int ci = 0, cj = 0;
-          if (!SPARSE && gm.graph_type != 0) { ci = a.cls[gb + i]; cj = a.cls[gb + j]; }
-          reinterpret_cast<int*>(tb + TBL_ROWOFF)[e] = (int)((gb + i) * 2 * H);
-          reinterpret_cast<int*>(tb + TBL_COLOFF)[e] = (int)((gb + j) * 2 * H + H);
+          if (!SPARSE && gm.graph_type != 0) { ci = a.cls[ge + i]; cj = a.cls[ge + j]; }
+          reinterpret_cast<int*>(tb + TBL_ROWOFF)[e] = (int)((ge + i) * 2 * H);
+          reinterpret_cast<int*>(tb + TBL_COLOFF)[e] = (int)((ge + j) * 2 * H + H);
           reinterpret_cast<float*>(tb + TBL_D)[e] = d;
           reinterpret_cast<float*>(tb + TBL_D0)[e] = d0;
-          const float bound = EMB ? a.ABmax[(gb + i) * 2] + a.ABmax[(gb + j) * 2 + 1] + a.wdmax
-                                  : a.ABmax[(gb + i) * 2] + a.ABmax[(gb + j) * 2 + 1] + d * a.wdmax + d0 * a.w0max;
+          const float bound = EMB ? a.ABmax[(ge + i) * 2] + a.ABmax[(ge + j) * 2 + 1] + a.wdmax
+                                  : a.ABmax[(ge + i) * 2] + a.ABmax[(ge + j) * 2 + 1] + d * a.wdmax + d0 * a.w0max;
           float sc = 1.0f;
           if (!(bound <= F16_TARGET)) {
             const int ex2 = ((__float_as_int(bound) >> 23) & 0xff) - 127;
@@ -391,7 +455,7 @@
           reinterpret_cast<float*>(tb + TBL_SC)[e] = sc;
           any_rescale |= (sc != 1.0f);
           const float ew = SPARSE ? ew_list
-                                  : edge_weight(gm.graph_type, a.edge_mask ? a.edge_mask + gb * N : nullptr, N, i, j, ci, cj, d0);
+                                  : edge_weight(gm.graph_type, a.edge_mask ? a.edge_mask + ge * N : nullptr, N, i, j, ci, cj, d0);
           reinterpret_cast<float2*>(tb + TBL_EM)[e] =
               COORD ? make_float2(ew, a.w2_descale / sc)
                     : make_float2(ew * -0.6931471805599453f, (a.w2_descale / sc) * -1.4426950408889634f);
@@ -414,6 +478,46 @@
     if (lane == 0) {
       mbar_expect_tx(bars + BAR_W, 2 * W_BYTES);
       bulk_g2s(sbase + OFF_WHI, w2tc, 2 * W_BYTES, bars + BAR_W);
+    }
+    if constexpr (COORD) {
+      float* carry = reinterpret_cast<float*>(sm + OFF_CARRY);
+      for (int t = 0;; ++t) {
+        const int acc = t & (N_ACC - 1), x = t % N_TX;
+        mbar_wait_relaxed(bars + BAR_TBL + 8 * acc, (t / N_ACC) & 1);
+        const uint8_t* tb = sm + OFF_TBL + acc * TBL_BYTES;
+        const int* hdr = reinterpret_cast<const int*>(tb + TBL_HDR);
+        if (hdr[0] <= 0) break;
+        mbar_wait_relaxed(bars + BAR_TXFULL + 8 * x, (t / N_TX) & 1);
+        const float* txs = reinterpret_cast<const float*>(sm + OFF_TX) + x * TN * 3;
+        const int nrt = hdr[1];
+        const bool first_chunk = hdr[3] & 1, last_chunk = hdr[3] & 2;
+        const size_t gb = (size_t)hdr[4] * N;
+        const int* rownode = reinterpret_cast<const int*>(tb + TBL_ROWNODE);
+        const int* rowstart = reinterpret_cast<const int*>(tb + TBL_ROWSTART);
+        const float cin = carry[lane & 3];
+        __syncwarp();
+        for (int p = lane; p < nrt * 3; p += 32) {
+          const int rr = p / 3, dim = p - rr * 3;
+          float sacc = (rr == 0 && !first_chunk) ? cin : 0.f;
+          const int col0 = rowstart[rr];
+          const int ncc = rowstart[rr + 1] - col0;
+          for (int jj = 0; jj < ncc; ++jj) sacc += txs[(col0 + jj) * 3 + dim];
+          if (rr == nrt - 1 && !last_chunk) {
+            carry[dim] = sacc;
+          } else {
+            const int i = rownode[rr];
+            const float lm = a.linker_mask ? a.linker_mask[gb + i] : 1.f;
+            const float xv = a.x[(gb + i) * 3 + dim];
+            float div = gm.normalization_factor;
+            if constexpr (MEAN) div = SPARSE ? (float)(hdr[6] > 0 ? hdr[6] : ncc) : (float)N;
+            const float xn = (xv + (sacc / div) * lm) * a.nm[gb + i];
+            a.x_out[(gb + i) * 3 + dim] = xn;
+            reinterpret_cast<float*>(a.x4_out + gb + i)[dim] = xn;
+          }
+        }
+        __syncwarp();
+        if (lane == 0) { mbar_arrive(bars + BAR_TXEMPTY + 8 * x); mbar_arrive(bars + BAR_TEMPTY + 8 * acc); }
+      }
     }
   }
   } else if (warp >= W_PROD) {
@@ -529,36 +633,32 @@
     const int g = warp >> 2;
     const int wq = warp & 3, q = lane & 3;
     const int r0 = 64 * g + 16 * wq + (lane >> 2);
-    float* txs = reinterpret_cast<float*>(sm + OFF_TX);
     float2 run = make_float2(0.f, 0.f);
-    float run3 = 0.f;
     float d[64];
 #pragma unroll
     for (int i = 0; i < 64; ++i) d[i] = 0.f;
     mbar_wait(bars + BAR_W, 0);
     for (int t = 0;; ++t) {
       const int acc = t & (N_ACC - 1), s = t & (N_STAGE - 1);
-      if (!COORD && g == 0 && t > 0) named_sync(BAR_TURN0, 32 * N_EPI_WARPS);
+      if (g == 0 && t > 0) named_sync(BAR_TURN0, 32 * N_EPI_WARPS);
       mbar_wait(bars + BAR_TBL + 8 * acc, (t / N_ACC) & 1);
       const uint8_t* tb = sm + OFF_TBL + acc * TBL_BYTES;
       const int* hdr = reinterpret_cast<const int*>(tb + TBL_HDR);
       const int Et = hdr[0];
       if (Et <= 0) break;
       const uint32_t bhi = sbase + OFF_ST + s * STAGE_BYTES, blo = bhi + B_BYTES;
-      if (!COORD) {
-        if (g == 1) named_sync(BAR_TURN1, 32 * N_EPI_WARPS);
-        mbar_wait(bars + BAR_FULL + 8 * s, (t / N_STAGE) & 1);
-        fence_acc(d);
-        wg_fence();
+      if (g == 1) named_sync(BAR_TURN1, 32 * N_EPI_WARPS);
+      mbar_wait(bars + BAR_FULL + 8 * s, (t / N_STAGE) & 1);
+      fence_acc(d);
+      wg_fence();
+      if (COORD)
+        mma_3xf16(d, bhi + g * 1024, blo + g * 1024, B_LBO, sbase + OFF_WHI, sbase + OFF_WLO, W_LBO, 2 * W_LBO, 8, false);
+      else
         mma_3xf16(d, sbase + OFF_WHI + g * 1024, sbase + OFF_WLO + g * 1024, W_LBO, bhi, blo, B_LBO, 2 * B_LBO, 8, false);
-        wg_commit();
-        named_arrive(g == 0 ? BAR_TURN1 : BAR_TURN0, 32 * N_EPI_WARPS);
-        wg_wait_all();
-        fence_acc(d);
-      } else {
-        mbar_wait(bars + BAR_FULL + 8 * s, (t / N_STAGE) & 1);
-        gemm_3xf16(d, bhi + g * 1024, blo + g * 1024, B_LBO, sbase + OFF_WHI, sbase + OFF_WLO, W_LBO, 2 * W_LBO, 8, false);
-      }
+      wg_commit();
+      named_arrive(g == 0 ? BAR_TURN1 : BAR_TURN0, 32 * N_EPI_WARPS);
+      wg_wait_all();
+      fence_acc(d);
       __syncwarp();
       if (lane == 0) mbar_arrive(bars + BAR_EMPTY + 8 * s);
 
@@ -646,6 +746,9 @@
         phia += __shfl_xor_sync(0xffffffffu, phia, 1); phib += __shfl_xor_sync(0xffffffffu, phib, 1);
         phia += __shfl_xor_sync(0xffffffffu, phia, 2); phib += __shfl_xor_sync(0xffffffffu, phib, 2);
         const float* cds = reinterpret_cast<const float*>(tb + TBL_CD);
+        const int x = t % N_TX;
+        if (t >= N_TX) mbar_wait(bars + BAR_TXEMPTY + 8 * x, ((t - N_TX) / N_TX) & 1);
+        float* txs = reinterpret_cast<float*>(sm + OFF_TX) + x * TN * 3;
         if constexpr (TANH) {
           const float range = a.coords_range;
           if (q == 0 && r0 < Et) {
@@ -670,27 +773,8 @@
             txs[e * 3 + 0] = cds[e * 3 + 0] * w; txs[e * 3 + 1] = cds[e * 3 + 1] * w; txs[e * 3 + 2] = cds[e * 3 + 2] * w;
           }
         }
-        named_sync(2, 32 * N_EPI_WARPS);
-        if (tid < nrt * 3) {
-          const int rr = tid / 3, dim = tid - rr * 3;
-          float sacc = (nrt == 1 && !first_chunk) ? run3 : 0.f;
-          const int col0 = rowstart[rr];
-          const int ncc = rowstart[rr + 1] - col0;
-          for (int jj = 0; jj < ncc; ++jj) sacc += txs[(col0 + jj) * 3 + dim];
-          if (nrt == 1) run3 = sacc;
-          if (last_chunk) {
-            const int i = rownode[rr];
-            const float lm = a.linker_mask ? a.linker_mask[gb + i] : 1.f;
-            const float xv = a.x[(gb + i) * 3 + dim];
-            float div = gm.normalization_factor;
-            if constexpr (MEAN) div = SPARSE ? (float)(hdr[6] > 0 ? hdr[6] : ncc) : (float)N;
-            const float xn = (xv + (sacc / div) * lm) * a.nm[gb + i];
-            a.x_out[(gb + i) * 3 + dim] = xn;
-            reinterpret_cast<float*>(a.x4_out + gb + i)[dim] = xn;
-          }
-        }
-        named_sync(2, 32 * N_EPI_WARPS);
-        if (lane == 0) mbar_arrive(bars + BAR_TEMPTY + 8 * acc);
+        __syncwarp();
+        if (lane == 0) mbar_arrive(bars + BAR_TXFULL + 8 * x);
       }
     }
   }
diff --git a/profiles/coord_update.py b/profiles/coord_update.py
--- /dev/null
+++ b/profiles/coord_update.py
@@ -0,0 +1,57 @@
+import argparse
+import json
+import os
+import statistics
+import subprocess
+import sys
+
+ROOT = os.path.dirname(os.path.dirname(os.path.abspath(__file__)))
+sys.path.insert(0, os.path.join(ROOT, "profiles"))
+from inpaint_sampling import card
+
+
+def kernel_table(tree, workload, reps):
+    env = dict(os.environ, DL_TIME_KERNELS="1")
+    out = subprocess.run([sys.executable, os.path.join(tree, "profiles", "time_kernels.py"), workload, str(reps)],
+                         cwd=tree, env=env, capture_output=True, text=True)
+    return (out.stdout + out.stderr).strip()
+
+
+def bench(tree, workload, steps):
+    out = subprocess.run([sys.executable, os.path.join(tree, "bench.py"), "--gpus", "1", "--steps", str(steps),
+                          "--warmup", "1", "--workload", workload, "--no-e2e", "--no-cpu-baseline"],
+                         cwd=tree, capture_output=True, text=True)
+    for line in reversed(out.stdout.splitlines()):
+        if line.startswith("{"):
+            r = json.loads(line)
+            return r["value"], statistics.median(r["loop_ms_device"]), r["gpu_launches"]
+    raise RuntimeError(f"bench.py in {tree} printed no result:\n{out.stdout[-2000:]}\n{out.stderr[-2000:]}")
+
+
+def main():
+    ap = argparse.ArgumentParser()
+    ap.add_argument("--old", required=True)
+    ap.add_argument("--workloads", default="cfg2_zinc,cfg2_zinc_ragged,cfg3_geom")
+    ap.add_argument("--reps", type=int, default=3)
+    ap.add_argument("--steps", type=int, default=3)
+    ap.add_argument("--forwards", type=int, default=20)
+    args = ap.parse_args()
+    trees = {"old": os.path.abspath(args.old), "new": ROOT}
+    for wl in args.workloads.split(","):
+        print(f"=== {wl}", flush=True)
+        for name, tree in trees.items():
+            print(f"--- kernel table, {name} build ({args.forwards} forwards)\n{kernel_table(tree, wl, args.forwards)}", flush=True)
+        runs = {name: [] for name in trees}
+        for _ in range(args.reps):
+            for name, tree in trees.items():
+                v, loop, launches = bench(tree, wl, args.steps)
+                runs[name].append(v)
+                print(f"{wl} {name}: {v:9.2f} molecules/s  loop {loop:8.1f} ms  {launches} launches", flush=True)
+        med = {n: statistics.median(r) for n, r in runs.items()}
+        print(f"{wl}: median old {med['old']:.2f}, new {med['new']:.2f} molecules/s ({100 * (med['new'] / med['old'] - 1):+.2f} %); "
+              f"old {min(runs['old']):.2f}-{max(runs['old']):.2f}, new {min(runs['new']):.2f}-{max(runs['new']):.2f}", flush=True)
+    print(f"card: {card()}")
+
+
+if __name__ == "__main__":
+    main()
```

New measurement: 191.8, median of 6. No clear change (+0.4%).
